# marl/l3embedding

Measured on AMD Instinct MI355X. Metric: AVC training pairs/sec (1s audio + 224x224 frame), higher is better.
Workload: dtype f32; 1 GPU; full cnn_L3_melspec2 AVC training step (audio+vision+fusion, fwd+bwd+Adam), batch 64 per GPU, global batch 64, fp32, inputs resident in HBM; global_batch=64, parallelism=dp1, fp32_conv=f4x4

## Files before the change

### include/l3hip.h

```cpp
#ifndef L3HIP_H
#define L3HIP_H

#include <stdint.h>

#ifdef __cplusplus
extern "C" {
#endif

#define L3_OK 0
#define L3_EINVAL (-1)
#define L3_EHIP (-2)
#define L3_ENOMEM (-3)
#define L3_ESTATE (-4)
#define L3_ECOMM (-5)

#define L3_MODEL_CNN_L3_ORIG 0
#define L3_MODEL_TINY_L3 1
#define L3_MODEL_CNN_L3_KAPREDBINPUTBN 2
#define L3_MODEL_CNN_L3_MELSPEC1 3
#define L3_MODEL_CNN_L3_MELSPEC2 4

typedef struct l3_engine l3_engine;

#define L3_DTYPE_F32 0
// ... 82 lines not shown
} l3_sample;
int l3_upload_batch_sampled(l3_engine *e, l3_clipbank *bank, const l3_sample *records, int n, int augment);
int l3_stage_batch_sampled(l3_engine *e, l3_clipbank *bank, const l3_sample *records, int n, int augment);
int l3_op_sample_batch(l3_clipbank *bank, const l3_sample *records, int n, int augment, uint8_t *out_u8, int16_t *out_i16,
                       double *gains);
int l3_step_forward(l3_engine *e, int training);
int l3_tower_step(l3_engine *e, int tower, int backward);
int l3_step_bucket_count(const l3_engine *e);
int l3_step_backward_bucket(l3_engine *e, int bucket);
int l3_step_update(l3_engine *e, float lr, float grad_scale);
int l3_step_resident(l3_engine *e, float lr);
int l3_step_results(l3_engine *e, float *loss, float *acc, float *probs, float *logits);
int l3_step_results_enqueue(l3_engine *e, int slot, int reduce);
int l3_step_results_wait(l3_engine *e, int slot, float *loss, float *acc);

int l3_replicas_upload(l3_engine *e, const float *video, const float *audio, const float *labels, int replicas);
int l3_replicas_upload_raw(l3_engine *e, const uint8_t *video_u8, const int16_t *audio_i16, const int32_t *labels_i32, int replicas);
int l3_replicas_upload_raw_aug(l3_engine *e, const uint8_t *video_u8, const int16_t *audio_i16, const int32_t *labels_i32,
                               const l3_augment_params *params, const double *u, int replicas);
int l3_replicas_stage_raw(l3_engine *e, const uint8_t *video_u8, const int16_t *audio_i16, const int32_t *labels_i32, int replicas);
int l3_replicas_stage_raw_aug(l3_engine *e, const uint8_t *video_u8, const int16_t *audio_i16, const int32_t *labels_i32,
                              const l3_augment_params *params, const double *u, int replicas);
int l3_step_replicas(l3_engine *e, float lr);
int l3_eval_replicas(l3_engine *e, float *loss, float *acc);

#define L3_COMM_ID_BYTES 128
int l3_comm_unique_id(void *id128);
int l3_comm_init(l3_engine *e, const void *id128, int world, int rank);
int l3_comm_destroy(l3_engine *e);
int l3_comm_info(const l3_engine *e, int *world, int *rank, char *library_path, int path_cap);
int l3_comm_version(void);
int l3_comm_allreduce_host(l3_engine *e, double *vals, int n, int op);
int l3_step_dp(l3_engine *e, float lr);
int l3_comm_timing(l3_engine *e, int on);
int l3_comm_timing_read(l3_engine *e, double *exposed_ms, double *span_ms, double *bucket_ms, int cap, int *steps);

int l3_grad_arena_dev(l3_engine *e, void **dev_ptr, int64_t *numel);
int l3_bucket_range(const l3_engine *e, int bucket, int64_t *offset, int64_t *numel);
int l3_bn_stats_pack_dev(l3_engine *e, void **send_dev, int64_t *numel);
int l3_bn_stats_replicas_dev(l3_engine *e, int world, void **gathered_dev);

int l3_embed_audio(l3_engine *e, const float *audio, int64_t n, int pool_h, int pool_w, float *out);
int l3_embed_vision(l3_engine *e, const float *video, int64_t n, int pool_h, int pool_w, float *out);
int64_t l3_embed_dim(const l3_engine *e, int vision, int pool_h, int pool_w);
int l3_embed_audio_frames(l3_engine *e, const float *samples, int64_t n_samples, const int64_t *table,
                          int64_t n_frames, int pool_h, int pool_w, float *out);
int l3_embed_audio_clips_resampled(l3_engine *e, const float *native, int64_t n_native, const int64_t *clips,
                                   int64_t n_clips, const double *half_window, int64_t n_window, int num_table,
                                   int64_t n_samples, const int64_t *table, int64_t n_frames, int pool_h, int pool_w,
                                   float *out);
int l3_embed_vision_frames(l3_engine *e, const uint8_t *pixels, int64_t n_bytes, const int64_t *table, int64_t n_frames,
                           int pool_h, int pool_w, float *out);

int l3_get_activation(l3_engine *e, const char *name, float *dst, int64_t numel);
int l3_activation_numel(l3_engine *e, const char *name, int64_t *numel);
int l3_sync(l3_engine *e);
int l3_profile_enable(l3_engine *e, int on);
int l3_set_tower_overlap(l3_engine *e, int on);
int l3_profile_read(l3_engine *e, int family, double *ms, int64_t *launches, double *flops);
int l3_profile_read_executed(l3_engine *e, int family, double *flops);
int l3_profile_read_bytes(l3_engine *e, int family, double *bytes);

#define L3_OP_BF16_STORED 2
#define L3_OP_BF16_STORED_OUT 3
int l3_op_conv2d_fwd_dt(int device, int dtype, const float *x, const float *w, const float *b, float *y,
                        int n, int h, int wd, int cin, int cout, int kh, int kw, int same);
int l3_op_conv2d_bwd_dt(int device, int dtype, const float *x, const float *w, const float *dy, float *dx,
                        float *dw, float *db, int n, int h, int wd, int cin, int cout, int kh, int kw, int same);
int l3_op_conv2d_fwd(int device, const float *x, const float *w, const float *b, float *y,
                     int n, int h, int wd, int cin, int cout, int kh, int kw, int same);
int l3_op_conv2d_bwd(int device, const float *x, const float *w, const float *dy,
                     float *dx, float *dw, float *db,
                     int n, int h, int wd, int cin, int cout, int kh, int kw, int same);
int l3_op_bn_relu_fwd(int device, const float *x, const float *gamma, const float *beta,
                      float *y, float *mean, float *var, int64_t rows, int c, int relu, int x_bf16);
int l3_op_bn_relu_bwd(int device, const float *x, const float *y, const float *dy,
                      const float *gamma, const float *beta, const float *mean, const float *var,
                      float *dx, float *dgamma, float *dbeta, int64_t rows, int c, int relu, int x_bf16);
int l3_op_bn_relu_pool2_fwd(int device, const float *x, const float *gamma, const float *beta, float *p,
                            float *mean, float *var, int n, int h, int wd, int c, int same, int relu_mode, int x_bf16);
int l3_op_bn_relu_pool2_bwd(int device, const float *x, const float *gamma, const float *beta, const float *dp,
                            float *dx, float *dgamma, float *dbeta, float *dbias, int n, int h, int wd, int c,
                            int same, int relu_mode, int x_bf16);
int l3_op_maxpool_fwd(int device, const float *x, float *y, int n, int h, int wd, int c,
                      int ph, int pw, int sh, int sw, int same);
int l3_op_maxpool_bwd(int device, const float *x, const float *dy, float *dx, int n, int h,
                      int wd, int c, int ph, int pw, int sh, int sw, int same);
int l3_op_frontend(int device, int model_type, const float *audio, int n, int db_max_scope, float *out);
int l3_op_frontend_form(int device, int model_type, int frontend, const float *audio, int n, float *out);
#define L3_FRONTEND_CFG_FIELDS 9
int l3_frontend_cfg(int t, int n_dft, int n_hop, int same, int n_mels, int32_t *cfg);
int l3_frontend_tables(const float *freq2mel, int n_mels, float *win, float *b1, float *b2, float *tw, int32_t *mel_start,
                       int32_t *mel_len, int32_t *mel_off, float *melw, int64_t melw_cap, int64_t *n_melw);
int l3_op_frontend_frames(int device, const float *audio, int b, int t, int n_dft, int n_hop, int pad_left, int n_frames,
                          float *frames, float *fe, float *fo, float *a1);
int l3_op_dft_twiddle(int device, const float *y, int frames, float *a2, float *nyq);
#define L3_SPEC_UNFOLDED 0
#define L3_SPEC_FOLDED 1
#define L3_SPEC_FACTORED 2
int l3_op_spec_to_features(int device, int layout, const float *spec, const float *nyq, int b, int n_frames, int n_dft, int n_mels,
                           const float *freq2mel, int flags, float *out);
int l3_op_dft_fused(int device, const float *audio, int b, int t, int n_hop, int pad_left, int n_frames, int n_mels,
                    const float *freq2mel, int flags, float *out);
int l3_op_db_normalize(int device, float *x, int b, int64_t per_sample, int batch_scope);
int l3_op_gather_frames(int device, const float *samples, int64_t n_samples, const int64_t *table,
                        int64_t n_frames, float *frames);
int l3_op_image_frames(int device, const uint8_t *pixels, int64_t n_bytes, const int64_t *table, int64_t n_frames,
                       uint8_t *out_u8, float *out_f32);
int l3_op_resample(int device, const float *x, int64_t n_in, int64_t sr_orig, int64_t sr_new, const double *half_window,
                   int64_t n_window, int num_table, int64_t t0, int64_t n_out, float *y);
int l3_op_resample_clips(int device, const float *x, int64_t n_in, const int64_t *clips, int64_t n_clips, int64_t sr_new,
                         const double *half_window, int64_t n_window, int num_table, int64_t n_samples, int copy_equal,
                         float *y);
int l3_op_bn_stats_from_partials(int device, const float *part, int nblk, int c, const float *pivot, int64_t rows,
                                 float eps, float *mean, float *var);
int l3_op_conv2d_fwd_stats(int device, int dtype, const float *x, const float *w, const float *b, float *y, float *part, int *nblk,
                           float *mean, float *var, int n, int h, int wd, int cin, int cout, int kh, int kw, int same,
                           int stat_mode);
int l3_op_conv2d_dgrad_bn_bwd(int device, int dtype, const float *dy, const float *w, const float *bn_x, const float *gamma,
                              const float *beta, const float *mean, const float *var, float *dx, float *part, int *nblk,
                              float *dgamma, float *dbeta, int n, int h, int wd, int cin, int cout, int kh, int kw, int same,
                              int relu, int64_t bn_rows);
int l3_op_first_block_bwd(int device, int form, int relu, const float *x, const float *gamma_in, const float *beta_in, const float *w,
                          const float *y, const float *gamma2, const float *beta2, const float *dA, float *mean_in, float *var_in,
                          float *xaug, float *mean2, float *var2, float *scale2, float *shift2, float *dgamma2, float *dbeta2,
                          float *coeffs, float *dY, float *gaug, float *dw, float *dbias, float *dgamma_in, float *dbeta_in, int n,
                          int h, int wd, int c, int cout);
int l3_op_first_conv_grads(int device, const float *gaug, const float *w, const float *gamma, const float *beta, float *dw,
                           float *dgamma, float *dbeta, float *dbias, int taps, int c, int co);
int l3_op_bn_relu_pool2_fwd_xwin(int device, const float *x, const float *gamma, const float *beta, float *p, float *mean,
                                 float *var, float *xwin, int n, int h, int wd, int c, int same, int relu_mode, int x_bf16);
int l3_op_preprocess(int device, const uint8_t *video_u8, int64_t nv, float *video,
                     const int16_t *audio_i16, int64_t na, float *audio);
int l3_op_augment_video(int device, const uint8_t *u8, int n, int h, int w, const l3_augment_params *params,
                        uint8_t *out_u8, float *out_f32);
int l3_op_augment_audio(int device, const int16_t *i16, int n, int t, const double *u, int16_t *out_i16, float *out_f32,
                        double *gains);

typedef struct l3_mlp l3_mlp;
int l3_mlp_create(int device, int D, int C, int batch, float weight_decay, uint64_t seed, l3_mlp **m);
void l3_mlp_destroy(l3_mlp *m);
int64_t l3_mlp_param_count(const l3_mlp *m);
int l3_mlp_set_data(l3_mlp *m, const float *X_train, const int32_t *y_train, int64_t n_train,
                    const float *X_valid, const int32_t *y_valid, int64_t n_valid);
int l3_mlp_epoch(l3_mlp *m, const int32_t *perm, float lr, int64_t t0, double *stats_out);
int l3_mlp_predict(l3_mlp *m, const float *X, int64_t n, float *probs_out);
int l3_mlp_get_weights(l3_mlp *m, float *dst, int64_t n);
int l3_mlp_set_weights(l3_mlp *m, const float *src, int64_t n);

int l3_op_mlp_dense_fwd(int device, const float *x, int64_t n_x, const int32_t *idx, int rows, int K, int N, const float *w,
                        const float *b, int relu, float *y);
int l3_op_mlp_dense_bwd_x(int device, const float *dy, const float *w, const float *h, int rows, int K, int N, float *dx);
int l3_op_mlp_wgrad(int device, const float *x, int64_t n_x, const int32_t *idx, int rows, int K, int N, const float *dy, float *dw,
                    float *db);
int l3_op_mlp_wgrad_adam(int device, const float *x, int64_t n_x, const int32_t *idx, int rows, int K, int N, const float *dy,
                         float *w, float *b, float *mw, float *vw, float *mb, float *vb, float weight_decay, float lr_t,
                         float *w2_out);
int l3_op_mlp_softmax_ce(int device, const float *z, const int32_t *labels, int rows, int C, float gscale, float *probs, float *dz,
                         float *ce, float *correct);
int l3_op_adam(int device, float *p, const float *g, float *m, float *v, int64_t n, int64_t n_l2, float l2x2, float lr_t);
int l3_op_adam_scaled(int device, float *p, const float *g, float *m, float *v, int64_t n, int64_t n_l2, float l2x2, float lr_t,
                      float b1, float b2, float eps, float gscale);
int l3_op_arena_fold(int device, float *acc, float *g, int64_t total, int64_t off, int64_t n, int mode);

int l3_op_head_dense_fwd(int device, const float *x, const float *w, const float *b, float *y, int B, int K, int N, int relu);
int l3_op_head_dense_bwd(int device, const float *x, const float *w, const float *dy, float *dw, float *db, float *dx, int B,
// ... 203 lines not shown
```

### l3embedding_amd/_lib.py

```python
import ctypes as C
import os

import numpy as np

from . import _build

MODEL_IDS = {
    'cnn_L3_orig': 0,
    'tiny_L3': 1,
    'cnn_L3_kapredbinputbn': 2,
    'cnn_L3_melspec1': 3,
    'cnn_L3_melspec2': 4,
}

FAMILIES = ('conv_fwd', 'conv_dgrad', 'conv_wgrad', 'elementwise', 'frontend', 'head', 'adam')


DTYPES = {'f32': 0, 'fp32': 0, 'float32': 0, 'bf16': 1}
FP32_CONV = {'f4x4': 0, 'f2x2': 1, 'f2x2_bf16x6': 2}
DP_MOVING = {'replicas': 0, 'rank_local': 1}
FRONTENDS = {'kapre': 0, 'minispec': 1}
OP_DTYPES = dict(DTYPES, bf16_stored=2, bf16_stored_out=3)


# ... 44 lines not shown
    'l3_reset_optimizer': (C.c_int, [C.c_void_p]),
    'l3_copy_state': (C.c_int, [C.c_void_p, C.c_void_p]),
    'l3_optimizer_steps': (C.c_int, [C.c_void_p, C.POINTER(C.c_int64), C.POINTER(C.c_int64)]),
    'l3_forward': (C.c_int, [C.c_void_p, C.c_void_p, C.c_void_p, C.c_int, C.c_void_p, C.c_void_p]),
    'l3_train_step': (C.c_int, [C.c_void_p, C.c_void_p, C.c_void_p, C.c_void_p, C.c_float,
                                C.POINTER(C.c_float), C.POINTER(C.c_float)]),
    'l3_eval_step': (C.c_int, [C.c_void_p, C.c_void_p, C.c_void_p, C.c_void_p,
                               C.POINTER(C.c_float), C.POINTER(C.c_float)]),
    'l3_upload_batch': (C.c_int, [C.c_void_p, C.c_void_p, C.c_void_p, C.c_void_p]),
    'l3_upload_batch_raw': (C.c_int, [C.c_void_p, C.c_void_p, C.c_void_p, C.c_void_p]),
    'l3_tower_step': (C.c_int, [C.c_void_p, C.c_int, C.c_int]),
    'l3_stage_batch_raw': (C.c_int, [C.c_void_p, C.c_void_p, C.c_void_p, C.c_void_p]),
    'l3_upload_batch_raw_aug': (C.c_int, [C.c_void_p, C.c_void_p, C.c_void_p, C.c_void_p, C.c_void_p, C.c_void_p]),
    'l3_stage_batch_raw_aug': (C.c_int, [C.c_void_p, C.c_void_p, C.c_void_p, C.c_void_p, C.c_void_p, C.c_void_p]),
    'l3_batch_gains': (C.c_int, [C.c_void_p, C.c_void_p]),
    'l3_clipbank_create': (C.c_int, [C.c_int, C.c_int64, C.c_int64, C.c_int, C.POINTER(C.c_void_p)]),
    'l3_clipbank_add': (C.c_int, [C.c_void_p, C.c_void_p, C.c_int, C.c_int, C.c_int, C.c_void_p, C.c_int64, C.c_int,
                                  C.POINTER(C.c_int)]),
    'l3_clipbank_info': (C.c_int, [C.c_void_p, C.c_int, C.c_void_p]),
    'l3_clipbank_audio': (C.c_int, [C.c_void_p, C.c_int, C.c_void_p]),
    'l3_clipbank_destroy': (None, [C.c_void_p]),
    'l3_upload_batch_sampled': (C.c_int, [C.c_void_p, C.c_void_p, C.c_void_p, C.c_int, C.c_int]),
    'l3_stage_batch_sampled': (C.c_int, [C.c_void_p, C.c_void_p, C.c_void_p, C.c_int, C.c_int]),
    'l3_op_sample_batch': (C.c_int, [C.c_void_p, C.c_void_p, C.c_int, C.c_int, C.c_void_p, C.c_void_p, C.c_void_p]),
    'l3_step_forward': (C.c_int, [C.c_void_p, C.c_int]),
    'l3_step_bucket_count': (C.c_int, [C.c_void_p]),
    'l3_step_backward_bucket': (C.c_int, [C.c_void_p, C.c_int]),
    'l3_step_update': (C.c_int, [C.c_void_p, C.c_float, C.c_float]),
    'l3_step_resident': (C.c_int, [C.c_void_p, C.c_float]),
    'l3_replicas_upload': (C.c_int, [C.c_void_p, C.c_void_p, C.c_void_p, C.c_void_p, C.c_int]),
    'l3_replicas_upload_raw': (C.c_int, [C.c_void_p, C.c_void_p, C.c_void_p, C.c_void_p, C.c_int]),
    'l3_replicas_stage_raw': (C.c_int, [C.c_void_p, C.c_void_p, C.c_void_p, C.c_void_p, C.c_int]),
    'l3_replicas_upload_raw_aug': (C.c_int, [C.c_void_p] * 6 + [C.c_int]),
    'l3_replicas_stage_raw_aug': (C.c_int, [C.c_void_p] * 6 + [C.c_int]),
    'l3_step_replicas': (C.c_int, [C.c_void_p, C.c_float]),
    'l3_eval_replicas': (C.c_int, [C.c_void_p, C.POINTER(C.c_float), C.POINTER(C.c_float)]),
    'l3_step_results': (C.c_int, [C.c_void_p, C.POINTER(C.c_float), C.POINTER(C.c_float), C.c_void_p, C.c_void_p]),
    'l3_step_results_enqueue': (C.c_int, [C.c_void_p, C.c_int, C.c_int]),
    'l3_step_results_wait': (C.c_int, [C.c_void_p, C.c_int, C.POINTER(C.c_float), C.POINTER(C.c_float)]),
    'l3_comm_unique_id': (C.c_int, [C.c_void_p]),
    'l3_comm_init': (C.c_int, [C.c_void_p, C.c_void_p, C.c_int, C.c_int]),
    'l3_comm_destroy': (C.c_int, [C.c_void_p]),
    'l3_comm_info': (C.c_int, [C.c_void_p, C.POINTER(C.c_int), C.POINTER(C.c_int), C.c_char_p, C.c_int]),
    'l3_comm_allreduce_host': (C.c_int, [C.c_void_p, C.POINTER(C.c_double), C.c_int, C.c_int]),
    'l3_step_dp': (C.c_int, [C.c_void_p, C.c_float]),
    'l3_comm_timing': (C.c_int, [C.c_void_p, C.c_int]),
    'l3_comm_timing_read': (C.c_int, [C.c_void_p, C.POINTER(C.c_double), C.POINTER(C.c_double), C.POINTER(C.c_double), C.c_int, C.POINTER(C.c_int)]),
    'l3_grad_arena_dev': (C.c_int, [C.c_void_p, C.POINTER(C.c_void_p), C.POINTER(C.c_int64)]),
    'l3_bucket_range': (C.c_int, [C.c_void_p, C.c_int, C.POINTER(C.c_int64), C.POINTER(C.c_int64)]),
    'l3_embed_audio': (C.c_int, [C.c_void_p, C.c_void_p, C.c_int64, C.c_int, C.c_int, C.c_void_p]),
    'l3_embed_vision': (C.c_int, [C.c_void_p, C.c_void_p, C.c_int64, C.c_int, C.c_int, C.c_void_p]),
    'l3_embed_dim': (C.c_int64, [C.c_void_p, C.c_int, C.c_int, C.c_int]),
    'l3_embed_audio_frames': (C.c_int, [C.c_void_p, C.c_void_p, C.c_int64, C.c_void_p, C.c_int64, C.c_int, C.c_int,
                                        C.c_void_p]),
    'l3_embed_audio_clips_resampled': (C.c_int, [C.c_void_p, C.c_void_p, C.c_int64, C.c_void_p, C.c_int64, C.c_void_p,
                                                 C.c_int64, C.c_int, C.c_int64, C.c_void_p, C.c_int64, C.c_int, C.c_int,
                                                 C.c_void_p]),
    'l3_embed_audio_frames_dev': (C.c_int, [C.c_void_p, C.c_void_p, C.c_int64, C.c_void_p, C.c_int64, C.c_int, C.c_int,
                                            C.c_void_p, C.c_int64]),
    'l3_embed_audio_clips_resampled_dev': (C.c_int, [C.c_void_p, C.c_void_p, C.c_int64, C.c_void_p, C.c_int64, C.c_void_p,
                                                     C.c_int64, C.c_int, C.c_int64, C.c_void_p, C.c_int64, C.c_int, C.c_int,
                                                     C.c_void_p, C.c_int64]),
    'l3_embed_vision_frames': (C.c_int, [C.c_void_p, C.c_void_p, C.c_int64, C.c_void_p, C.c_int64, C.c_int, C.c_int,
                                         C.c_void_p]),
    'l3_embed_vision_frames_dev': (C.c_int, [C.c_void_p, C.c_void_p, C.c_int64, C.c_void_p, C.c_int64, C.c_int, C.c_int,
                                             C.c_void_p, C.c_int64]),
    'l3_get_activation': (C.c_int, [C.c_void_p, C.c_char_p, C.c_void_p, C.c_int64]),
    'l3_activation_numel': (C.c_int, [C.c_void_p, C.c_char_p, C.POINTER(C.c_int64)]),
    'l3_sync': (C.c_int, [C.c_void_p]),
    'l3_profile_enable': (C.c_int, [C.c_void_p, C.c_int]),
    'l3_set_tower_overlap': (C.c_int, [C.c_void_p, C.c_int]),
    'l3_profile_read_executed': (C.c_int, [C.c_void_p, C.c_int, C.POINTER(C.c_double)]),
    'l3_profile_read_bytes': (C.c_int, [C.c_void_p, C.c_int, C.POINTER(C.c_double)]),
    'l3_profile_read': (C.c_int, [C.c_void_p, C.c_int, C.POINTER(C.c_double), C.POINTER(C.c_int64),
                                  C.POINTER(C.c_double)]),
    'l3_op_conv2d_fwd': (C.c_int, [C.c_int, C.c_void_p, C.c_void_p, C.c_void_p, C.c_void_p] + [C.c_int] * 8),
    'l3_op_conv2d_fwd_dt': (C.c_int, [C.c_int, C.c_int, C.c_void_p, C.c_void_p, C.c_void_p, C.c_void_p] + [C.c_int] * 8),
    'l3_op_conv2d_bwd_dt': (C.c_int, [C.c_int, C.c_int] + [C.c_void_p] * 6 + [C.c_int] * 8),
    'l3_op_conv2d_bwd': (C.c_int, [C.c_int] + [C.c_void_p] * 6 + [C.c_int] * 8),
    'l3_op_bn_relu_fwd': (C.c_int, [C.c_int] + [C.c_void_p] * 6 + [C.c_int64, C.c_int, C.c_int, C.c_int]),
    'l3_op_bn_relu_bwd': (C.c_int, [C.c_int] + [C.c_void_p] * 10 + [C.c_int64, C.c_int, C.c_int, C.c_int]),
    'l3_op_bn_relu_pool2_fwd': (C.c_int, [C.c_int] + [C.c_void_p] * 6 + [C.c_int] * 7),
    'l3_op_bn_relu_pool2_bwd': (C.c_int, [C.c_int] + [C.c_void_p] * 8 + [C.c_int] * 7),
    'l3_op_maxpool_fwd': (C.c_int, [C.c_int, C.c_void_p, C.c_void_p] + [C.c_int] * 9),
    'l3_op_maxpool_bwd': (C.c_int, [C.c_int, C.c_void_p, C.c_void_p, C.c_void_p] + [C.c_int] * 9),
    'l3_op_frontend': (C.c_int, [C.c_int, C.c_int, C.c_void_p, C.c_int, C.c_int, C.c_void_p]),
    'l3_op_frontend_form': (C.c_int, [C.c_int, C.c_int, C.c_int, C.c_void_p, C.c_int, C.c_void_p]),
    'l3_spectrogram_shape': (C.c_int, [C.c_void_p, C.c_void_p, C.c_void_p]),
    'l3_audio_spectrograms': (C.c_int, [C.c_void_p, C.c_void_p, C.c_int64, C.c_void_p, C.c_int64, C.c_void_p]),
    'l3_embed_audio_spec': (C.c_int, [C.c_void_p, C.c_void_p, C.c_int64, C.c_int, C.c_int, C.c_void_p]),
    'l3_embed_audio_spec_dev': (C.c_int, [C.c_void_p, C.c_void_p, C.c_int64, C.c_int, C.c_int, C.c_void_p, C.c_int64]),
    'l3_tower_dim': (C.c_int, [C.c_void_p, C.c_int]),
    'l3_tower_features': (C.c_int, [C.c_void_p, C.c_int, C.c_void_p, C.c_int64, C.c_void_p]),
    'l3_tower_features_dev': (C.c_int, [C.c_void_p, C.c_int, C.c_void_p, C.c_int64, C.c_void_p, C.c_int64]),
    'l3_tower_features_sampled_dev': (C.c_int, [C.c_void_p, C.c_void_p, C.c_void_p, C.c_int64, C.c_void_p, C.c_void_p, C.c_int64]),
    'l3_pairs_create': (C.c_int, [C.c_int, C.c_int, C.c_int, C.c_int, C.POINTER(C.c_void_p)]),
    'l3_pairs_destroy': (None, [C.c_void_p]),
    'l3_pairs_set_head': (C.c_int, [C.c_void_p] * 5),
    'l3_pairs_set_vision': (C.c_int, [C.c_void_p, C.c_void_p, C.c_int64]),
    'l3_pairs_set_audio': (C.c_int, [C.c_void_p, C.c_void_p, C.c_int64]),
    'l3_pairs_set_vision_dev': (C.c_int, [C.c_void_p, C.c_void_p, C.c_int64, C.c_int64]),
    'l3_pairs_set_audio_dev': (C.c_int, [C.c_void_p, C.c_void_p, C.c_int64, C.c_int64]),
    'l3_pairs_matrix': (C.c_int, [C.c_void_p] + [C.c_int64] * 4 + [C.c_int, C.c_void_p]),
    'l3_pairs_list': (C.c_int, [C.c_void_p, C.c_void_p, C.c_void_p, C.c_int64, C.c_void_p]),
    'l3_pairs_ranks': (C.c_int, [C.c_void_p] * 7),
    'l3_pairs_time': (C.c_int, [C.c_void_p, C.c_int, C.c_int64, C.c_int, C.POINTER(C.c_double)]),
    'l3_op_project': (C.c_int, [C.c_int, C.c_void_p, C.c_void_p, C.c_void_p, C.c_int64, C.c_int, C.c_int, C.c_void_p]),
    'l3_op_pair_margins': (C.c_int, [C.c_int, C.c_void_p, C.c_void_p, C.c_void_p, C.c_float, C.c_int64, C.c_int64, C.c_int, C.c_void_p]),
    'l3_frontend_cfg': (C.c_int, [C.c_int] * 5 + [C.c_void_p]),
    'l3_frontend_tables': (C.c_int, [C.c_void_p, C.c_int] + [C.c_void_p] * 8 + [C.c_int64, C.POINTER(C.c_int64)]),
    'l3_op_frontend_frames': (C.c_int, [C.c_int, C.c_void_p] + [C.c_int] * 6 + [C.c_void_p] * 4),
    'l3_op_dft_twiddle': (C.c_int, [C.c_int, C.c_void_p, C.c_int, C.c_void_p, C.c_void_p]),
    'l3_op_spec_to_features': (C.c_int, [C.c_int, C.c_int, C.c_void_p, C.c_void_p] + [C.c_int] * 4 + [C.c_void_p, C.c_int, C.c_void_p]),
    'l3_op_dft_fused': (C.c_int, [C.c_int, C.c_void_p] + [C.c_int] * 6 + [C.c_void_p, C.c_int, C.c_void_p]),
    'l3_op_db_normalize': (C.c_int, [C.c_int, C.c_void_p, C.c_int, C.c_int64, C.c_int]),
    'l3_op_gather_frames': (C.c_int, [C.c_int, C.c_void_p, C.c_int64, C.c_void_p, C.c_int64, C.c_void_p]),
    'l3_op_image_frames': (C.c_int, [C.c_int, C.c_void_p, C.c_int64, C.c_void_p, C.c_int64, C.c_void_p, C.c_void_p]),
    'l3_op_resample': (C.c_int, [C.c_int, C.c_void_p, C.c_int64, C.c_int64, C.c_int64, C.c_void_p, C.c_int64, C.c_int,
                                 C.c_int64, C.c_int64, C.c_void_p]),
    'l3_op_resample_clips': (C.c_int, [C.c_int, C.c_void_p, C.c_int64, C.c_void_p, C.c_int64, C.c_int64, C.c_void_p, C.c_int64,
                                       C.c_int, C.c_int64, C.c_int, C.c_void_p]),
    'l3_op_bn_stats_from_partials': (C.c_int, [C.c_int, C.c_void_p, C.c_int, C.c_int, C.c_void_p, C.c_int64, C.c_float,
                                               C.c_void_p, C.c_void_p]),
    'l3_op_conv2d_fwd_stats': (C.c_int, [C.c_int, C.c_int] + [C.c_void_p] * 5 + [C.POINTER(C.c_int), C.c_void_p, C.c_void_p] +
                               [C.c_int] * 9),
    'l3_op_conv2d_dgrad_bn_bwd': (C.c_int, [C.c_int, C.c_int] + [C.c_void_p] * 9 + [C.POINTER(C.c_int), C.c_void_p, C.c_void_p] +
                                  [C.c_int] * 9 + [C.c_int64]),
    'l3_op_first_block_bwd': (C.c_int, [C.c_int] * 3 + [C.c_void_p] * 24 + [C.c_int] * 5),
    'l3_op_first_conv_grads': (C.c_int, [C.c_int] + [C.c_void_p] * 8 + [C.c_int] * 3),
    'l3_op_bn_relu_pool2_fwd_xwin': (C.c_int, [C.c_int] + [C.c_void_p] * 7 + [C.c_int] * 7),
    'l3_op_preprocess': (C.c_int, [C.c_int, C.c_void_p, C.c_int64, C.c_void_p, C.c_void_p, C.c_int64, C.c_void_p]),
    'l3_op_augment_video': (C.c_int, [C.c_int, C.c_void_p, C.c_int, C.c_int, C.c_int, C.c_void_p, C.c_void_p, C.c_void_p]),
    'l3_op_augment_audio': (C.c_int, [C.c_int, C.c_void_p, C.c_int, C.c_int, C.c_void_p, C.c_void_p, C.c_void_p, C.c_void_p]),
    'l3_mlp_create': (C.c_int, [C.c_int, C.c_int, C.c_int, C.c_int, C.c_float, C.c_uint64, C.POINTER(C.c_void_p)]),
    'l3_mlp_destroy': (None, [C.c_void_p]),
    'l3_mlp_param_count': (C.c_int64, [C.c_void_p]),
    'l3_mlp_set_data': (C.c_int, [C.c_void_p, C.c_void_p, C.c_void_p, C.c_int64, C.c_void_p, C.c_void_p, C.c_int64]),
    'l3_mlp_epoch': (C.c_int, [C.c_void_p, C.c_void_p, C.c_float, C.c_int64, C.POINTER(C.c_double)]),
    'l3_mlp_predict': (C.c_int, [C.c_void_p, C.c_void_p, C.c_int64, C.c_void_p]),
    'l3_mlp_get_weights': (C.c_int, [C.c_void_p, C.c_void_p, C.c_int64]),
    'l3_mlp_set_weights': (C.c_int, [C.c_void_p, C.c_void_p, C.c_int64]),
    'l3_op_mlp_dense_fwd': (C.c_int, [C.c_int, C.c_void_p, C.c_int64, C.c_void_p, C.c_int, C.c_int, C.c_int, C.c_void_p,
                                      C.c_void_p, C.c_int, C.c_void_p]),
    'l3_op_mlp_dense_bwd_x': (C.c_int, [C.c_int, C.c_void_p, C.c_void_p, C.c_void_p, C.c_int, C.c_int, C.c_int, C.c_void_p]),
    'l3_op_mlp_wgrad': (C.c_int, [C.c_int, C.c_void_p, C.c_int64, C.c_void_p, C.c_int, C.c_int, C.c_int, C.c_void_p,
                                  C.c_void_p, C.c_void_p]),
    'l3_op_mlp_wgrad_adam': (C.c_int, [C.c_int, C.c_void_p, C.c_int64, C.c_void_p, C.c_int, C.c_int, C.c_int, C.c_void_p]
                             + [C.c_void_p] * 6 + [C.c_float, C.c_float, C.c_void_p]),
    'l3_op_mlp_softmax_ce': (C.c_int, [C.c_int, C.c_void_p, C.c_void_p, C.c_int, C.c_int, C.c_float] + [C.c_void_p] * 4),
    'l3_op_adam': (C.c_int, [C.c_int] + [C.c_void_p] * 4 + [C.c_int64, C.c_int64, C.c_float, C.c_float]),
    'l3_op_adam_scaled': (C.c_int, [C.c_int] + [C.c_void_p] * 4 + [C.c_int64, C.c_int64] + [C.c_float] * 6),
    'l3_op_arena_fold': (C.c_int, [C.c_int, C.c_void_p, C.c_void_p, C.c_int64, C.c_int64, C.c_int64, C.c_int]),
    'l3_op_head_dense_fwd': (C.c_int, [C.c_int] + [C.c_void_p] * 4 + [C.c_int] * 4),
    'l3_op_head_dense_bwd': (C.c_int, [C.c_int] + [C.c_void_p] * 6 + [C.c_int] * 3),
    'l3_op_softmax_ce2': (C.c_int, [C.c_int, C.c_void_p, C.c_void_p, C.c_int, C.c_float] + [C.c_void_p] * 3),
    'l3_op_sumsq': (C.c_int, [C.c_int, C.c_void_p, C.c_int64, C.c_void_p, C.c_void_p, C.c_int, C.c_int, C.c_void_p]),
    'l3_op_bn_moving_update': (C.c_int, [C.c_int, C.c_int, C.c_void_p, C.c_void_p, C.c_int64] + [C.c_void_p] * 4
                               + [C.c_int64, C.c_int, C.c_int64, C.c_float, C.c_int, C.c_int64, C.c_void_p, C.c_int64]),
    'l3_svm_create': (C.c_int, [C.c_int, C.POINTER(C.c_void_p)]),
    'l3_svm_destroy': (None, [C.c_void_p]),
    'l3_svm_set_data': (C.c_int, [C.c_void_p, C.c_void_p, C.c_int64, C.c_int]),
    'l3_svm_fit': (C.c_int, [C.c_void_p, C.c_void_p, C.c_double, C.c_double, C.c_int64, C.c_int] + [C.c_void_p] * 3
                   + [C.c_int] + [C.c_void_p] * 5),
    'l3_svm_fit_costs': (C.c_int, [C.c_void_p, C.c_void_p, C.c_void_p, C.c_double, C.c_int64, C.c_int] + [C.c_void_p] * 3
                         + [C.c_int] + [C.c_void_p] * 5),
    'l3_svm_cv_decision': (C.c_int, [C.c_void_p, C.c_void_p, C.c_int] + [C.c_void_p] * 8),
# ... 689 lines not shown
    for k in ('mean2', 'var2', 'scale2', 'shift2', 'dgamma2', 'dbeta2'):
        out[k] = np.empty(co, f32)
    coeffs = np.empty((3, co), f32) if form != 'explicit' else None
    dY = np.empty_like(y) if form == 'explicit' else None
    out.update(gaug=np.empty((9, c + 1, co), f32), dw=np.empty((3, 3, c, co), f32), dbias=np.empty(co, f32),
               dgamma_in=np.empty(c, f32), dbeta_in=np.empty(c, f32))
    names = ('mean_in', 'var_in', 'xaug', 'mean2', 'var2', 'scale2', 'shift2', 'dgamma2', 'dbeta2')
    tail = ('gaug', 'dw', 'dbias', 'dgamma_in', 'dbeta_in')
    check(lib.l3_op_first_block_bwd(device, FIRST_BLOCK_FORMS[form], int(relu), _ptr(x), _ptr(vin[0]), _ptr(vin[1]), _ptr(w), _ptr(y),
                                    _ptr(v2[0]), _ptr(v2[1]), _ptr(dA), *([_ptr(out[k]) for k in names] + [_ptr(coeffs), _ptr(dY)] +
                                                                          [_ptr(out[k]) for k in tail] + [n, h, wd, c, co])))
    if dY is not None:
        out['dY'] = dY
    else:
        out['cA'], out['cB'], out['cC'] = coeffs
    return out


def op_first_conv_grads(gaug, w, gamma, beta, want_dbias=True, device=0):
    lib = load()
    gaug, w, gamma, beta = _f32(gaug), _f32(w), _f32(gamma), _f32(beta)
    taps, c, co = w.shape
    assert gaug.shape == (taps, c + 1, co) and gamma.shape == (c,) and beta.shape == (c,)
    dw = np.empty_like(w)
    dg, db = np.empty(c, np.float32), np.empty(c, np.float32)
    dbias = np.empty(co, np.float32) if want_dbias else None
    check(lib.l3_op_first_conv_grads(device, _ptr(gaug), _ptr(w), _ptr(gamma), _ptr(beta), _ptr(dw), _ptr(dg), _ptr(db), _ptr(dbias),
                                     taps, c, co))
    return dw, dg, db, dbias


def op_bn_relu_fwd(x, gamma, beta, relu, device=0, x_bf16=False, out_bf16=False):
    lib = load()
    x = _f32(x)
    c = x.shape[-1]
    rows = x.size // c
    y = np.empty_like(x)
    mean, var = np.empty((c,), np.float32), np.empty((c,), np.float32)
    check(lib.l3_op_bn_relu_fwd(device, _ptr(x), _ptr(_f32(gamma)), _ptr(_f32(beta)), _ptr(y), _ptr(mean),
                                _ptr(var), rows, c, int(relu), int(x_bf16) | (4 if out_bf16 else 0)))
    return y, mean, var


def op_bn_relu_bwd(x, y, dy, gamma, mean, var, relu, device=0, beta=None, x_bf16=False, out_bf16=False):
    lib = load()
    x, y, dy = _f32(x), _f32(y), _f32(dy)
    c = x.shape[-1]
    rows = x.size // c
    dx = np.empty_like(x)
    dg, db = np.empty((c,), np.float32), np.empty((c,), np.float32)
    check(lib.l3_op_bn_relu_bwd(device, _ptr(x), _ptr(y), _ptr(dy), _ptr(_f32(gamma)), _ptr(_f32(beta)), _ptr(_f32(mean)),
                                _ptr(_f32(var)), _ptr(dx), _ptr(dg), _ptr(db), rows, c, int(relu), int(x_bf16) | (4 if out_bf16 else 0)))
    return dx, dg, db


def op_bn_relu_pool2_fwd(x, gamma, beta, same, device=0, relu_mode=1, x_bf16=False, want_xwin=False, out_bf16=False):
    lib = load()
    flags = int(x_bf16) | (4 if out_bf16 else 0)
    x = _f32(x)
    n, h, wd, c = x.shape
    p = np.empty((n, _pool_out(h, 2, 2, same), _pool_out(wd, 2, 2, same), c), np.float32)
    mean, var = np.empty((c,), np.float32), np.empty((c,), np.float32)
    if want_xwin:
        xwin = np.empty_like(p)
        check(lib.l3_op_bn_relu_pool2_fwd_xwin(device, _ptr(x), _ptr(_f32(gamma)), _ptr(_f32(beta)), _ptr(p), _ptr(mean), _ptr(var),
                                               _ptr(xwin), n, h, wd, c, int(same), int(relu_mode), flags))
        return p, mean, var, xwin
    check(lib.l3_op_bn_relu_pool2_fwd(device, _ptr(x), _ptr(_f32(gamma)), _ptr(_f32(beta)), _ptr(p), _ptr(mean),
                                      _ptr(var), n, h, wd, c, int(same), int(relu_mode), flags))
    return p, mean, var


def op_bn_relu_pool2_bwd(x, gamma, beta, dp, same, device=0, relu_mode=1, x_bf16=False, out_bf16=False):
    lib = load()
    x, dp = _f32(x), _f32(dp)
    n, h, wd, c = x.shape
    dx = np.empty_like(x)
    dg, db, dbias = (np.empty((c,), np.float32) for _ in range(3))
    check(lib.l3_op_bn_relu_pool2_bwd(device, _ptr(x), _ptr(_f32(gamma)), _ptr(_f32(beta)), _ptr(dp), _ptr(dx),
                                      _ptr(dg), _ptr(db), _ptr(dbias), n, h, wd, c, int(same), int(relu_mode), int(x_bf16) | (4 if out_bf16 else 0)))
    return dx, dg, db, dbias


def _pool_out(h, p, s, same):
    return -(-h // s) if same else (h - p) // s + 1


def op_maxpool_fwd(x, ph, pw, sh, sw, same, device=0):
    lib = load()
    x = _f32(x)
    n, h, wd, c = x.shape
    y = np.empty((n, _pool_out(h, ph, sh, same), _pool_out(wd, pw, sw, same), c), np.float32)
    check(lib.l3_op_maxpool_fwd(device, _ptr(x), _ptr(y), n, h, wd, c, ph, pw, sh, sw, int(same)))
    return y


def op_maxpool_bwd(x, dy, ph, pw, sh, sw, same, device=0):
    lib = load()
    x, dy = _f32(x), _f32(dy)
    n, h, wd, c = x.shape
    dx = np.empty_like(x)
    check(lib.l3_op_maxpool_bwd(device, _ptr(x), _ptr(dy), _ptr(dx), n, h, wd, c, ph, pw, sh, sw, int(same)))
    return dx


def op_bn_stats_from_partials(part, pivot, rows, eps=1e-3, device=0):
    lib = load()
    part, pivot = _f32(part), _f32(pivot)
    nblk, two, c = part.shape
    assert two == 2 and pivot.shape == (c,)
    mean, var = np.empty(c, np.float32), np.empty(c, np.float32)
    check(lib.l3_op_bn_stats_from_partials(device, _ptr(part), nblk, c, _ptr(pivot), int(rows), float(eps), _ptr(mean), _ptr(var)))
    return mean, var


def op_frontend(model_type, audio, db_max_scope='sample', device=0):
    lib = load()
    a = _f32(audio)
    n = a.shape[0]
    probe = {'cnn_L3_orig': (257, 197), 'tiny_L3': (257, 198), 'cnn_L3_kapredbinputbn': (257, 197),
             'cnn_L3_melspec1': (128, 199), 'cnn_L3_melspec2': (256, 199)}[model_type]
    out = np.empty((n, probe[0], probe[1], 1), np.float32)
    check(lib.l3_op_frontend(device, MODEL_IDS[model_type], _ptr(a), n, 0 if db_max_scope == 'sample' else 1, _ptr(out)))
    return out


def op_frontend_form(model_type, audio, frontend='minispec', device=0):
    lib = load()
    a = _f32(audio)
    n = a.shape[0]
    f, frames = {'cnn_L3_orig': (257, 197), 'tiny_L3': (257, 198), 'cnn_L3_kapredbinputbn': (257, 197),
                 'cnn_L3_melspec1': (128, 199), 'cnn_L3_melspec2': (256, 199)}[model_type]
    if frontend == 'minispec':
        frames = 199
    out = np.empty((n, f, frames, 1), np.float32)
    check(lib.l3_op_frontend_form(device, MODEL_IDS[model_type], FRONTENDS[frontend], _ptr(a), n, _ptr(out)))
    return out


FRONTEND_CFG_FIELDS = ('n_frames', 'pad_left', 'n_freq', 'ncols_pad', 'ke', 'ko', 'nc', 'N1', 'N2')
SPEC_LAYOUTS = dict(unfolded=0, folded=1, factored=2)


def frontend_cfg(t, n_dft, n_hop, same, n_mels=0):
    v = np.zeros(len(FRONTEND_CFG_FIELDS), np.int32)
    check(load().l3_frontend_cfg(int(t), int(n_dft), int(n_hop), int(bool(same)), int(n_mels), _ptr(v)))
    return dict(zip(FRONTEND_CFG_FIELDS, (int(x) for x in v)))


def frontend_tables(n_mels=0, freq2mel=None):
    f32 = np.float32
    out = dict(win=np.empty(2048, f32), b1=np.empty((32, 64), f32), b2=np.empty((128, 64), f32), tw=np.empty((64, 32, 2), f32))
    fb = _f32(freq2mel)
    assert fb is None or fb.shape == (1025, n_mels)
    st, ln, of = (np.zeros(n_mels, np.int32) for _ in range(3))
    cap = 1025 * max(n_mels, 1)
    melw = np.empty(cap, f32)
    n = C.c_int64(0)
    check(load().l3_frontend_tables(_ptr(fb), int(n_mels), _ptr(out['win']), _ptr(out['b1']), _ptr(out['b2']), _ptr(out['tw']), _ptr(st),
                                    _ptr(ln), _ptr(of), _ptr(melw), cap, C.byref(n)))
    if n_mels:
        out.update(mel_start=st, mel_len=ln, mel_off=of, melw=melw[:n.value].copy())
    return out


def op_frontend_frames(audio, n_dft, n_hop, pad_left, n_frames, device=0):
# ... 1368 lines not shown
```

### l3embedding_amd/csrc/bn_fused.hip

```cpp
#include "kernels.h"
#include "device_common.h"

namespace l3 {



__device__ __forceinline__ void store_quad(void* base, int64_t q, f32x4 v, int obf) {
    if (obf) {
        bf16x4 h;
        h[0] = (__bf16)v.x; h[1] = (__bf16)v.y; h[2] = (__bf16)v.z; h[3] = (__bf16)v.w;
        __builtin_nontemporal_store(h, reinterpret_cast<bf16x4*>(base) + q);
    } else {
        __builtin_nontemporal_store(v, reinterpret_cast<f32x4*>(base) + q);
    }
}

template <bool XBF>
__device__ __forceinline__ f32x4 load_quad(const void* base, int64_t q) {
    if constexpr (XBF) {
        const u32x2 r = __builtin_nontemporal_load(reinterpret_cast<const u32x2*>(base) + q);
        return f32x4{__uint_as_float(r.x << 16), __uint_as_float(r.x & 0xffff0000u), __uint_as_float(r.y << 16),
                     __uint_as_float(r.y & 0xffff0000u)};
    } else {
        return __builtin_nontemporal_load(reinterpret_cast<const f32x4*>(base) + q);
// ... 236 lines not shown
template <bool XBF, bool WIN>
__global__ __launch_bounds__(FB) void bn_relu_pool2_fwd_kernel(const void* __restrict__ x, const f32x4* scale, const f32x4* shift,
                                                              void* __restrict__ p, Pool2Geom g, int mode, int obf, void* __restrict__ xwin) {
    constexpr int U = 2;
    const int64_t total = (int64_t)g.N * g.Ho * g.Wo * g.C4;
    const int c4 = (int)threadIdx.x % g.C4;
    const f32x4 sc = scale[c4], sh = shift[c4];
    const int64_t stride = (int64_t)gridDim.x * (FB * U);
    for (int64_t q = (int64_t)blockIdx.x * (FB * U) + threadIdx.x; q < total; q += stride) {
        f32x4 xs[U][4];
        int64_t po[U], wo_[U];
        bool w1[U], h1[U], live[U];
#pragma unroll
        for (int u = 0; u < U; ++u) {
            live[u] = q + u * FB < total;
            int n = 0, ho = 0, wo = 0;
            pool_index(g, live[u] ? q + u * FB : q, g.Ho, g.Wo, n, ho, wo);
            const int h0 = 2 * ho, w0 = 2 * wo;
            h1[u] = h0 + 1 < g.H; w1[u] = w0 + 1 < g.W;
            const int64_t base = ((int64_t)(n * g.H + h0) * g.W + w0) * g.C4 + c4;
            const int64_t dw = w1[u] ? g.C4 : 0, dh = h1[u] ? (int64_t)g.W * g.C4 : 0;
            xs[u][0] = load_quad<XBF>(x, base); xs[u][1] = load_quad<XBF>(x, base + dw);
            xs[u][2] = load_quad<XBF>(x, base + dh); xs[u][3] = load_quad<XBF>(x, base + dh + dw);
            po[u] = (int64_t)n * g.out_bs4 + ((int64_t)ho * g.Wo + wo) * g.C4 + c4;
            wo_[u] = ((int64_t)(n * g.Ho + ho) * g.Wo + wo) * g.C4 + c4;
        }
#pragma unroll
        for (int u = 0; u < U; ++u) {
            if (!live[u]) continue;
            f32x4 x00 = xs[u][0], x01 = xs[u][1], x10 = xs[u][2], x11 = xs[u][3];
            const bool h1ok = h1[u], w1ok = w1[u];
            if (mode == 2) { x00 = relu4(x00); x01 = relu4(x01); x10 = relu4(x10); x11 = relu4(x11); }
            const f32x4 v00 = bn_pre(x00, sc, sh), v01 = bn_pre(x01, sc, sh);
            const f32x4 v10 = bn_pre(x10, sc, sh), v11 = bn_pre(x11, sc, sh);
            f32x4 m;
            m.x = fmaxf(fmaxf(v00.x, v01.x), fmaxf(v10.x, v11.x));
            m.y = fmaxf(fmaxf(v00.y, v01.y), fmaxf(v10.y, v11.y));
            m.z = fmaxf(fmaxf(v00.z, v01.z), fmaxf(v10.z, v11.z));
            m.w = fmaxf(fmaxf(v00.w, v01.w), fmaxf(v10.w, v11.w));
            if (mode == 1) m = relu4(m);
            store_quad(p, po[u], m, obf);
            if constexpr (WIN) {
                const f32x4 r00 = mode == 1 ? relu4(v00) : v00, r01 = mode == 1 ? relu4(v01) : v01;
                const f32x4 r10 = mode == 1 ? relu4(v10) : v10, r11 = mode == 1 ? relu4(v11) : v11;
                const bool ok11 = h1ok && w1ok;
                f32x4 xw;
#define L3_WIN(comp)                                                                                  \
    {                                                                                                 \
        const int k = argmax4(r00.comp, r01.comp, r10.comp, r11.comp, w1ok, h1ok, ok11);              \
        xw.comp = k == 0 ? x00.comp : k == 1 ? x01.comp : k == 2 ? x10.comp : x11.comp;               \
    }
                L3_WIN(x) L3_WIN(y) L3_WIN(z) L3_WIN(w)
#undef L3_WIN
                store_quad(xwin, wo_[u], xw, XBF ? 1 : 0);
            }
        }
    }
}

static Pool2Geom make_pool2(int N, int H, int W, int C, int Ho, int Wo, int64_t out_batch_stride) {
    Pool2Geom g;
    g.N = N; g.H = H; g.W = W; g.C4 = C / 4; g.Ho = Ho; g.Wo = Wo;
    g.Hc = (H + 1) / 2; g.Wc = (W + 1) / 2;
    g.out_bs4 = out_batch_stride / 4;
    g.lgC4 = 0;
    while ((1 << g.lgC4) < g.C4) ++g.lgC4;
    g.small = (int64_t)N * g.Hc * g.Wc < ((int64_t)1 << 31) && (int64_t)N * H * W < ((int64_t)1 << 31);
    return g;
}

void bn_relu_pool2_fwd(const float* x, const float* scale, const float* shift, float* p, int N, int H, int W, int C,
                       int Ho, int Wo, int64_t out_batch_stride, int mode, hipStream_t s, int out_bf16, int x_bf16, void* xwin) {
    const Pool2Geom g = make_pool2(N, H, W, C, Ho, Wo, out_batch_stride);
    const int64_t total = (int64_t)N * Ho * Wo * g.C4;
    int64_t nb = (total + FB * 2 - 1) / (FB * 2);
    if (nb > 65536) nb = 65536;
    if (nb < 1) nb = 1;
    auto k = xwin != nullptr ? (x_bf16 ? bn_relu_pool2_fwd_kernel<true, true> : bn_relu_pool2_fwd_kernel<false, true>)
                             : (x_bf16 ? bn_relu_pool2_fwd_kernel<true, false> : bn_relu_pool2_fwd_kernel<false, false>);
    hipLaunchKernelGGL(k, dim3((int)nb), dim3(FB), 0, s, (const void*)x, reinterpret_cast<const f32x4*>(scale),
                       reinterpret_cast<const f32x4*>(shift), (void*)p, g, mode, out_bf16, xwin);
}

struct BwdCoef {
    float *A, *B, *Cc;
};

template <bool POOL, bool XBF, bool DYBF>
__global__ __launch_bounds__(FB) void bn_bwd_reduce_fast_kernel(const void* x, const void* dy, const f32x4* scale,
                                                               const f32x4* shift, const f32x4* mean,
                                                               const f32x4* var, float* part, int64_t n4,
                                                               Pool2Geom g, float eps, int relu) {
    const int64_t q0 = (int64_t)blockIdx.x * FB + threadIdx.x;
    const int c4 = (int)(q0 % g.C4);
    const f32x4 sc = scale[c4], sh = shift[c4], mu = mean[c4];
    const f32x4 vv = var[c4];
    const f32x4 rs = {rsqrtf(vv.x + eps), rsqrtf(vv.y + eps), rsqrtf(vv.z + eps), rsqrtf(vv.w + eps)};
    f32x4 a0 = {0.f, 0.f, 0.f, 0.f}, a1 = {0.f, 0.f, 0.f, 0.f};
    const int64_t stride = (int64_t)gridDim.x * FB;
    if constexpr (!POOL) {
        for (int64_t q = q0; q < n4; q += stride) {
            f32x4 xv = load_quad<XBF>(x, q);
            f32x4 d = load_quad<DYBF>(dy, q);
            if (relu == 1) {
                const f32x4 pre = bn_pre(xv, sc, sh);
                d.x = pre.x > 0.f ? d.x : 0.f; d.y = pre.y > 0.f ? d.y : 0.f;
                d.z = pre.z > 0.f ? d.z : 0.f; d.w = pre.w > 0.f ? d.w : 0.f;
            } else if (relu == 2) {
                xv = relu4(xv);
            }
            a0 += d;
            a1 += d * ((xv - mu) * rs);
        }
    } else {
        const int64_t total = (int64_t)g.N * g.Ho * g.Wo * g.C4;
        for (int64_t q = q0; q < total; q += stride) {
            int n, ho, wo;
            pool_index(g, q, g.Ho, g.Wo, n, ho, wo);
            const int h0 = 2 * ho, w0 = 2 * wo;
            const bool h1ok = h0 + 1 < g.H, w1ok = w0 + 1 < g.W;
            const int64_t base = ((int64_t)(n * g.H + h0) * g.W + w0) * g.C4 + c4;
            const int64_t dw = w1ok ? g.C4 : 0, dh = h1ok ? (int64_t)g.W * g.C4 : 0;
            f32x4 x00 = load_quad<XBF>(x, base), x01 = load_quad<XBF>(x, base + dw), x10 = load_quad<XBF>(x, base + dh),
                  x11 = load_quad<XBF>(x, base + dh + dw);
            if (relu == 2) { x00 = relu4(x00); x01 = relu4(x01); x10 = relu4(x10); x11 = relu4(x11); }
            f32x4 p00 = bn_pre(x00, sc, sh), p01 = bn_pre(x01, sc, sh), p10 = bn_pre(x10, sc, sh),
                  p11 = bn_pre(x11, sc, sh);
            const float gate = relu == 2 ? -INFINITY : 0.f;
            if (relu != 2) { p00 = relu4(p00); p01 = relu4(p01); p10 = relu4(p10); p11 = relu4(p11); }
            const f32x4 dp = load_quad<DYBF>(dy, (int64_t)n * g.out_bs4 + ((int64_t)ho * g.Wo + wo) * g.C4 + c4);
            const bool ok11 = h1ok && w1ok;
#define L3_RED(comp)                                                                                      \
    {                                                                                                     \
        const int k = argmax4(p00.comp, p01.comp, p10.comp, p11.comp, w1ok, h1ok, ok11);                  \
        const float pk = k == 0 ? p00.comp : k == 1 ? p01.comp : k == 2 ? p10.comp : p11.comp;            \
        const float xk = k == 0 ? x00.comp : k == 1 ? x01.comp : k == 2 ? x10.comp : x11.comp;            \
        const float d = pk > gate ? dp.comp : 0.f;                                                        \
        a0.comp += d;                                                                                     \
        a1.comp += d * ((xk - mu.comp) * rs.comp);                                                        \
    }
            L3_RED(x) L3_RED(y) L3_RED(z) L3_RED(w)
#undef L3_RED
        }
    }
    block_write_partials(a0, a1, part, g.C4);
}

struct BwdFinal {
    const float* gamma;
    const float* mean;
    const float* var;
    float *dgamma, *dbeta, *A, *B, *Cc;
    double inv_n;
    float eps;
    int training;
    __device__ void operator()(int c, double s0, double s1) const {
        dbeta[c] = (float)s0;
        dgamma[c] = (float)s1;
        const double rstd = 1.0 / sqrt((double)var[c] + (double)eps);
        const double gr = (double)gamma[c] * rstd;
        A[c] = (float)gr;
        if (training) {
            B[c] = (float)(-gr * rstd * s1 * inv_n);
            Cc[c] = (float)(gr * (-s0 * inv_n + (double)mean[c] * rstd * s1 * inv_n));
        } else {
            B[c] = 0.f;
            Cc[c] = 0.f;
        }
    }
};

template <bool POOL, bool XBF, bool DYBF>
__global__ __launch_bounds__(FB) void bn_bwd_apply_fast_kernel(const void* x, const void* dy, const f32x4* scale,
                                                              const f32x4* shift, const f32x4* cA, const f32x4* cB,
                                                              const f32x4* cC, void* dx, float* part, int64_t n4,
                                                              Pool2Geom g, int relu, int obf) {
    const int64_t q0 = (int64_t)blockIdx.x * FB + threadIdx.x;
    const int c4 = (int)(q0 % g.C4);
    const f32x4 sc = scale[c4], sh = shift[c4], A = cA[c4], B = cB[c4], Cc = cC[c4];
    f32x4 a0 = {0.f, 0.f, 0.f, 0.f};
    const int64_t stride = (int64_t)gridDim.x * FB;
    if constexpr (!POOL) {
        for (int64_t q = q0; q < n4; q += stride) {
            const f32x4 xr = load_quad<XBF>(x, q);
            f32x4 xv = xr;
            f32x4 d = load_quad<DYBF>(dy, q);
            if (relu == 1) {
                const f32x4 pre = bn_pre(xv, sc, sh);
                d.x = pre.x > 0.f ? d.x : 0.f; d.y = pre.y > 0.f ? d.y : 0.f;
                d.z = pre.z > 0.f ? d.z : 0.f; d.w = pre.w > 0.f ? d.w : 0.f;
            } else if (relu == 2) {
                xv = relu4(xv);
            }
            f32x4 o = A * d + (B * xv + Cc);
            if (relu == 2) {
                o.x = xr.x > 0.f ? o.x : 0.f; o.y = xr.y > 0.f ? o.y : 0.f;
                o.z = xr.z > 0.f ? o.z : 0.f; o.w = xr.w > 0.f ? o.w : 0.f;
            }
            store_quad(dx, q, o, obf);
            a0 += o;
        }
    } else {
        constexpr int U = XBF ? 2 : 1;
        const int64_t total = (int64_t)g.N * g.Hc * g.Wc * g.C4;
        for (int64_t q = (int64_t)blockIdx.x * (FB * U) + threadIdx.x; q < total; q += stride * U) {
            f32x4 rs[U][4], dps[U];
            int64_t bases[U];
            bool w1[U], h1[U], lives[U], on[U];
#pragma unroll
            for (int u = 0; u < U; ++u) {
                on[u] = q + u * FB < total;
                int n, hc, wc;
                pool_index(g, on[u] ? q + u * FB : q, g.Hc, g.Wc, n, hc, wc);
                const int h0 = 2 * hc, w0 = 2 * wc;
                h1[u] = h0 + 1 < g.H; w1[u] = w0 + 1 < g.W;
                lives[u] = hc < g.Ho && wc < g.Wo;
                const int64_t base = ((int64_t)(n * g.H + h0) * g.W + w0) * g.C4 + c4;
                const int64_t dw = w1[u] ? g.C4 : 0, dh = h1[u] ? (int64_t)g.W * g.C4 : 0;
                bases[u] = base;
                rs[u][0] = load_quad<XBF>(x, base); rs[u][1] = load_quad<XBF>(x, base + dw);
                rs[u][2] = load_quad<XBF>(x, base + dh); rs[u][3] = load_quad<XBF>(x, base + dh + dw);
                dps[u] = f32x4{0.f, 0.f, 0.f, 0.f};
                if (lives[u]) dps[u] = load_quad<DYBF>(dy, (int64_t)n * g.out_bs4 + ((int64_t)hc * g.Wo + wc) * g.C4 + c4);
            }
#pragma unroll
            for (int u = 0; u < U; ++u) {
                if (!on[u]) continue;
                const bool h1ok = h1[u], w1ok = w1[u], live = lives[u];
                const int64_t base = bases[u];
                const int64_t dw = w1ok ? g.C4 : 0, dh = h1ok ? (int64_t)g.W * g.C4 : 0;
                const f32x4 r00 = rs[u][0], r01 = rs[u][1], r10 = rs[u][2], r11 = rs[u][3];
                f32x4 x00 = r00, x01 = r01, x10 = r10, x11 = r11;
                if (relu == 2) { x00 = relu4(x00); x01 = relu4(x01); x10 = relu4(x10); x11 = relu4(x11); }
                f32x4 d00 = {0.f, 0.f, 0.f, 0.f}, d01 = d00, d10 = d00, d11 = d00;
                if (live) {
                    f32x4 p00 = bn_pre(x00, sc, sh), p01 = bn_pre(x01, sc, sh), p10 = bn_pre(x10, sc, sh),
                          p11 = bn_pre(x11, sc, sh);
                    const float gate = relu == 2 ? -INFINITY : 0.f;
                    if (relu != 2) { p00 = relu4(p00); p01 = relu4(p01); p10 = relu4(p10); p11 = relu4(p11); }
                    const f32x4 dp = dps[u];
                    const bool ok11 = h1ok && w1ok;
#define L3_APP(comp)                                                                                      \
    {                                                                                                     \
        const int k = argmax4(p00.comp, p01.comp, p10.comp, p11.comp, w1ok, h1ok, ok11);                  \
        const float pk = k == 0 ? p00.comp : k == 1 ? p01.comp : k == 2 ? p10.comp : p11.comp;            \
        const float d = pk > gate ? dp.comp : 0.f;                                                        \
        d00.comp = k == 0 ? d : 0.f;                                                                      \
        d01.comp = k == 1 ? d : 0.f;                                                                      \
        d10.comp = k == 2 ? d : 0.f;                                                                      \
        d11.comp = k == 3 ? d : 0.f;                                                                      \
    }
                    L3_APP(x) L3_APP(y) L3_APP(z) L3_APP(w)
#undef L3_APP
                }
                auto gate2 = [&](f32x4 o, f32x4 r) {
                    if (relu == 2) {
                        o.x = r.x > 0.f ? o.x : 0.f; o.y = r.y > 0.f ? o.y : 0.f;
                        o.z = r.z > 0.f ? o.z : 0.f; o.w = r.w > 0.f ? o.w : 0.f;
                    }
                    return o;
                };
                const f32x4 o00 = gate2(A * d00 + (B * x00 + Cc), r00);
                store_quad(dx, base, o00, obf);
                a0 += o00;
                if (w1ok) {
                    const f32x4 o = gate2(A * d01 + (B * x01 + Cc), r01);
                    store_quad(dx, base + dw, o, obf);
                    a0 += o;
                }
                if (h1ok) {
                    const f32x4 o = gate2(A * d10 + (B * x10 + Cc), r10);
                    store_quad(dx, base + dh, o, obf);
                    a0 += o;
                }
                if (h1ok && w1ok) {
                    const f32x4 o = gate2(A * d11 + (B * x11 + Cc), r11);
                    store_quad(dx, base + dh + dw, o, obf);
                    a0 += o;
                }
            }
        }
    }
    if (part != nullptr) block_write_partials(a0, a0, part, g.C4);
}

struct SumFinal {
    float* out;
    __device__ void operator()(int c, double s0, double) const { out[c] = (float)s0; }
};

void bn_bwd_fast(const float* x, const float* scale, const float* shift, const float* mean, const float* var,
                 const float* gamma, const float* dy, int pooled, int N, int H, int W, int C, int Ho, int Wo,
                 int64_t dy_batch_stride, float* dx, float* dgamma, float* dbeta, float* dbias, float* scratch,
                 float eps, int relu, int training, hipStream_t s, int dx_bf16, int x_bf16, int dy_bf16,
                 const float* ready_part, int ready_blocks) {
    const int64_t rows = (int64_t)N * H * W;
    const int64_t n4 = rows * (C / 4);
    Pool2Geom g = make_pool2(N, H, W, C, pooled ? Ho : H, pooled ? Wo : W, pooled ? dy_batch_stride : (int64_t)H * W * C);
    float* part = scratch;
    float* cA = scratch + (size_t)FAST_MAX_BLOCKS * 2 * C;
    float* cB = cA + C;
    float* cC = cB + C;
    const void* xv = (const void*)x;
    const void* dyv = (const void*)dy;
    const f32x4* sc4 = reinterpret_cast<const f32x4*>(scale);
    const f32x4* sh4 = reinterpret_cast<const f32x4*>(shift);
    const int64_t work_r = pooled ? (int64_t)N * Ho * Wo * (C / 4) : n4;
    const int nb_r = fast_blocks(work_r);
    const int variant = (pooled ? 4 : 0) | (x_bf16 ? 2 : 0) | (dy_bf16 ? 1 : 0);
    using ReduceFn = void (*)(const void*, const void*, const f32x4*, const f32x4*, const f32x4*, const f32x4*, float*, int64_t,
                              Pool2Geom, float, int);
    static const ReduceFn reduce_fns[8] = {
        bn_bwd_reduce_fast_kernel<false, false, false>, bn_bwd_reduce_fast_kernel<false, false, true>,
        bn_bwd_reduce_fast_kernel<false, true, false>,  bn_bwd_reduce_fast_kernel<false, true, true>,
        bn_bwd_reduce_fast_kernel<true, false, false>,  bn_bwd_reduce_fast_kernel<true, false, true>,
        bn_bwd_reduce_fast_kernel<true, true, false>,   bn_bwd_reduce_fast_kernel<true, true, true>};
    if (ready_part != nullptr) {
        launch_fast_final(BwdFinal{gamma, mean, var, dgamma, dbeta, cA, cB, cC, 1.0 / (double)rows, eps, training}, ready_part,
                          ready_blocks, C, s);
    } else {
        hipLaunchKernelGGL(reduce_fns[variant], dim3(nb_r), dim3(FB), 0, s, xv, dyv, sc4, sh4, reinterpret_cast<const f32x4*>(mean),
                           reinterpret_cast<const f32x4*>(var), part, n4, g, eps, relu);
        launch_fast_final(BwdFinal{gamma, mean, var, dgamma, dbeta, cA, cB, cC, 1.0 / (double)rows, eps, training}, part,
                          nb_r, C, s);
    }
    if (dx == nullptr) return;
    const int64_t work_a = pooled ? (int64_t)N * g.Hc * g.Wc * (C / 4) : n4;
    const int nb_a = fast_blocks(work_a);
    float* part2 = dbias ? part : nullptr;
    using ApplyFn = void (*)(const void*, const void*, const f32x4*, const f32x4*, const f32x4*, const f32x4*, const f32x4*, void*,
                             float*, int64_t, Pool2Geom, int, int);
    static const ApplyFn apply_fns[8] = {
        bn_bwd_apply_fast_kernel<false, false, false>, bn_bwd_apply_fast_kernel<false, false, true>,
        bn_bwd_apply_fast_kernel<false, true, false>,  bn_bwd_apply_fast_kernel<false, true, true>,
        bn_bwd_apply_fast_kernel<true, false, false>,  bn_bwd_apply_fast_kernel<true, false, true>,
        bn_bwd_apply_fast_kernel<true, true, false>,   bn_bwd_apply_fast_kernel<true, true, true>};
    hipLaunchKernelGGL(apply_fns[variant], dim3(nb_a), dim3(FB), 0, s, xv, dyv, sc4, sh4, reinterpret_cast<const f32x4*>(cA),
                       reinterpret_cast<const f32x4*>(cB), reinterpret_cast<const f32x4*>(cC), (void*)dx, part2, n4, g, relu,
                       dx_bf16);
    if (dbias) launch_fast_final(SumFinal{dbias}, part, nb_a, C, s);
}

}
```

### l3embedding_amd/csrc/elementwise.hip

```cpp
#include <algorithm>

#include "kernels.h"

namespace l3 {

static constexpr int RED_BLOCK = 256;
static constexpr int RED_MAX_BLOCKS = 1024;
static constexpr int SMALLC_MAX = 16;

static inline int red_blocks(int64_t rows, int C) {
    int rows_per_pass = (C % 4 == 0 && C >= 4 && C <= 1024) ? (RED_BLOCK / (C / 4) > 0 ? RED_BLOCK / (C / 4) : 1) : RED_BLOCK;
    int64_t b = (rows + (int64_t)rows_per_pass * 16 - 1) / ((int64_t)rows_per_pass * 16);
    if (b < 1) b = 1;
    if (b > RED_MAX_BLOCKS) b = RED_MAX_BLOCKS;
    return (int)b;
}

size_t colreduce_scratch_floats(int64_t rows, int C) {
    const size_t a = (size_t)red_blocks(rows, C) * 2 * (size_t)(C < 4 ? 4 : C) + 64;
    const size_t b = bn_fast_ok(C) ? bn_fast_scratch_floats(C) : 0;
    return a > b ? a : b;
}

template <class F>
// ... 446 lines not shown
}
typedef float gp4 __attribute__((ext_vector_type(4)));
__device__ __forceinline__ void gp_scan(const float* __restrict__ xb, int P, int C, int pg, float best[4], int arg[4]) {
#pragma unroll
    for (int e = 0; e < 4; ++e) {
        best[e] = -INFINITY;
        arg[e] = 0x7fffffff;
    }
    for (int p = pg; p < P; p += 16) {
        const gp4 v = *reinterpret_cast<const gp4*>(xb + (size_t)p * C);
#pragma unroll
        for (int e = 0; e < 4; ++e)
            if (v[e] > best[e] || arg[e] == 0x7fffffff) {
                best[e] = v[e];
                arg[e] = p;
            }
    }
}
__device__ __forceinline__ void gp_merge(float (*sb)[64], int (*sa)[64], int pg, int cq, float best[4], int arg[4]) {
#pragma unroll
    for (int e = 0; e < 4; ++e) {
        sb[pg][cq * 4 + e] = best[e];
        sa[pg][cq * 4 + e] = arg[e];
    }
    __syncthreads();
    if (pg == 0) {
#pragma unroll
        for (int e = 0; e < 4; ++e) {
            float b = best[e];
            int a = arg[e];
            for (int k = 1; k < 16; ++k) {
                const float vb = sb[k][cq * 4 + e];
                const int va = sa[k][cq * 4 + e];
                if (vb > b || (vb == b && va < a)) {
                    b = vb;
                    a = va;
                }
            }
            sb[0][cq * 4 + e] = b;
            sa[0][cq * 4 + e] = a;
        }
    }
    __syncthreads();
}
__global__ __launch_bounds__(256) void global_maxpool_fwd_kernel(const float* __restrict__ x, float* __restrict__ y, int P,
                                                                 int C, int64_t out_batch_stride) {
    __shared__ float sb[16][64];
    __shared__ int sa[16][64];
    const int cb = blockIdx.x % (C / 64), n = blockIdx.x / (C / 64);
    const int cq = threadIdx.x & 15, pg = threadIdx.x >> 4;
    float best[4];
    int arg[4];
    gp_scan(x + (size_t)n * P * C + cb * 64 + cq * 4, P, C, pg, best, arg);
    gp_merge(sb, sa, pg, cq, best, arg);
    if (threadIdx.x < 64) y[(size_t)n * out_batch_stride + cb * 64 + threadIdx.x] = sb[0][threadIdx.x];
}
__global__ __launch_bounds__(256) void global_maxpool_bwd_kernel(const float* __restrict__ x, const float* __restrict__ dy,
                                                                 float* __restrict__ dx, int P, int C,
                                                                 int64_t out_batch_stride) {
    __shared__ float sb[16][64];
    __shared__ int sa[16][64];
    const int cb = blockIdx.x % (C / 64), n = blockIdx.x / (C / 64);
    const int cq = threadIdx.x & 15, pg = threadIdx.x >> 4;
    float best[4];
    int arg[4];
    const size_t base = (size_t)n * P * C + cb * 64 + cq * 4;
    gp_scan(x + base, P, C, pg, best, arg);
    gp_merge(sb, sa, pg, cq, best, arg);
    const gp4 d = *reinterpret_cast<const gp4*>(dy + (size_t)n * out_batch_stride + cb * 64 + cq * 4);
    int am[4];
#pragma unroll
    for (int e = 0; e < 4; ++e) am[e] = sa[0][cq * 4 + e];
    for (int p = pg; p < P; p += 16) {
        gp4 o;
#pragma unroll
        for (int e = 0; e < 4; ++e) o[e] = p == am[e] ? d[e] : 0.f;
        *reinterpret_cast<gp4*>(dx + base + (size_t)p * C) = o;
    }
}
static bool is_global_pool(const PoolGeom& g) {
    return g.Ho == 1 && g.Wo == 1 && g.padT == 0 && g.padL == 0 && g.ph == g.H && g.pw == g.W && g.C % 64 == 0 &&
           g.out_batch_stride % 4 == 0;
}

void maxpool_fwd(const float* x, float* y, const PoolGeom& g, hipStream_t s) {
    if (is_global_pool(g)) {
        hipLaunchKernelGGL(global_maxpool_fwd_kernel, dim3(g.N * (g.C / 64)), dim3(256), 0, s, x, y, g.H * g.W, g.C,
                           (int64_t)g.out_batch_stride);
        return;
    }
    const int64_t total = (int64_t)g.N * g.Ho * g.Wo * g.C;
    hipLaunchKernelGGL(maxpool_fwd_kernel, dim3(ew_blocks(total)), dim3(256), 0, s, x, y, g);
}
__global__ __launch_bounds__(256) void maxpool_bwd_kernel(const float* x, const float* dy, float* dx, PoolGeom g) {
    const int64_t total = (int64_t)g.N * g.Ho * g.Wo * g.C;
    for (int64_t i = (int64_t)blockIdx.x * 256 + threadIdx.x; i < total; i += (int64_t)gridDim.x * 256) {
        const int c = (int)(i % g.C);
        int64_t r = i / g.C;
        const int wo = (int)(r % g.Wo);
        r /= g.Wo;
        const int ho = (int)(r % g.Ho);
        const int n = (int)(r / g.Ho);
        const int h0 = ho * g.sh - g.padT, w0 = wo * g.sw - g.padL;
        float best = -INFINITY;
        int ba = -1, bb = -1;
        for (int a = 0; a < g.ph; ++a) {
            const int h = h0 + a;
            if ((unsigned)h >= (unsigned)g.H) continue;
            for (int b = 0; b < g.pw; ++b) {
                const int w = w0 + b;
                if ((unsigned)w >= (unsigned)g.W) continue;
                const float v = x[((size_t)(n * g.H + h) * g.W + w) * g.C + c];
                if (ba < 0 || v > best) { best = v; ba = a; bb = b; }
            }
        }
        const float d = dy[(size_t)n * g.out_batch_stride + ((size_t)ho * g.Wo + wo) * g.C + c];
        for (int a = 0; a < g.ph; ++a) {
            const int h = h0 + a;
            if ((unsigned)h >= (unsigned)g.H) continue;
            for (int b = 0; b < g.pw; ++b) {
                const int w = w0 + b;
                if ((unsigned)w >= (unsigned)g.W) continue;
                dx[((size_t)(n * g.H + h) * g.W + w) * g.C + c] = (a == ba && b == bb) ? d : 0.f;
            }
        }
    }
}
void maxpool_bwd(const float* x, const float* dy, float* dx, const PoolGeom& g, hipStream_t s) {
    if (is_global_pool(g)) {
        hipLaunchKernelGGL(global_maxpool_bwd_kernel, dim3(g.N * (g.C / 64)), dim3(256), 0, s, x, dy, dx, g.H * g.W,
                           g.C, (int64_t)g.out_batch_stride);
        return;
    }
    const bool covers = (g.Ho - 1) * g.sh - g.padT + g.ph >= g.H && (g.Wo - 1) * g.sw - g.padL + g.pw >= g.W &&
                        g.sh == g.ph && g.sw == g.pw;
    if (!covers) (void)hipMemsetAsync(dx, 0, (size_t)g.N * g.H * g.W * g.C * sizeof(float), s);
    const int64_t total = (int64_t)g.N * g.Ho * g.Wo * g.C;
    hipLaunchKernelGGL(maxpool_bwd_kernel, dim3(ew_blocks(total)), dim3(256), 0, s, x, dy, dx, g);
}

__global__ __launch_bounds__(256) void bn_xhat_ones_kernel(const float* __restrict__ x, const float* __restrict__ mean,
                                                           const float* __restrict__ var, float eps, float* __restrict__ xa,
                                                           int64_t rows, int C) {
    const int C1 = C + 1;
    const int64_t total = rows * C1;
    for (int64_t i = (int64_t)blockIdx.x * 256 + threadIdx.x; i < total; i += (int64_t)gridDim.x * 256) {
        const int c = (int)(i % C1);
        const int64_t r = i / C1;
        xa[i] = c == C ? 1.f : (x[r * C + c] - mean[c]) * (1.f / sqrtf(var[c] + eps));
    }
}
void bn_xhat_ones(const float* x, const float* mean, const float* var, float eps, float* xa, int64_t rows, int C,
                  hipStream_t s) {
    hipLaunchKernelGGL(bn_xhat_ones_kernel, dim3(ew_blocks(rows * (C + 1))), dim3(256), 0, s, x, mean, var, eps, xa, rows, C);
}

__global__ __launch_bounds__(256) void first_conv_grads_kernel(const float* __restrict__ gaug, const float* __restrict__ w,
                                                               const float* __restrict__ gamma, const float* __restrict__ beta,
                                                               float* __restrict__ dw, float* __restrict__ dgamma,
                                                               float* __restrict__ dbeta, float* __restrict__ dbias, int taps,
                                                               int C, int Co) {
    __shared__ double red[2][256];
    const int t = threadIdx.x;
    const int C1 = C + 1;
    for (int i = t; i < taps * C * Co; i += 256) {
        const int co = i % Co, ci = (i / Co) % C, tap = i / (Co * C);
// ... 324 lines not shown
```

### l3embedding_amd/csrc/engine.hip

```cpp
#include <hip/hip_runtime.h>
#include "knobs.h"

#include <cmath>
#include <cstdio>
#include <cstdlib>
#include <cstring>
#include <map>
#include <string>
#include <vector>

#include "../../include/l3hip.h"
#include "comm.h"
#include "conv_path.h"
#include "featprep.h"
#include "kernels.h"

namespace {

using namespace l3;

static thread_local std::string g_create_error;

constexpr float BN_EPS = 1e-3f;
constexpr float BN_MOMENTUM = 0.99f;
constexpr float L2_WEIGHT = 1e-5f;
constexpr float ADAM_B1 = 0.9f, ADAM_B2 = 0.999f, ADAM_EPS = 1e-8f;
constexpr int AUDIO_T = 48000;

enum ParamKind { PK_KERNEL, PK_BIAS, PK_GAMMA, PK_BETA, PK_MMEAN, PK_MVAR, PK_CONST };
enum OpKind { OP_CONV, OP_BN, OP_RELU, OP_POOL, OP_FLATTEN };
enum Family { F_CONV_FWD, F_CONV_DGRAD, F_CONV_WGRAD, F_ELEMWISE, F_FRONTEND, F_HEAD, F_ADAM, F_COUNT };

struct Tensor {
    float* d = nullptr;
    float* g = nullptr;
    int N = 0, H = 0, W = 0, C = 0;
    int64_t batch_stride = 0;
    bool alias = false;
    bool d_bf16 = false, g_bf16 = false;
    int64_t numel() const { return (int64_t)N * H * W * C; }
    int64_t rows() const { return (int64_t)N * H * W; }
};

struct Param {
    std::string name;
    int ndim = 0;
    int64_t shape[4] = {1, 1, 1, 1};
    bool trainable = false;
    int kind = 0;
    int64_t numel = 0;
    int bucket = 0;
    float* d = nullptr;
    float* g = nullptr;
};

enum FirstWgrad { FW_NONE, FW_AUG, FW_AUG_DEFERRED };
struct ConvPlan {
    ConvStorage st;
    ConvFwdPath fwd;
    int stat_mode = 0;
    FirstWgrad aug = FW_NONE;
    ConvWgradPath wgrad;
    bool colsum = false;
    ConvDgradPath dgrad;
    int bwd_bn = -1;
    double fwd_bytes = 0.0, wg_bytes = 0.0, dg_bytes = 0.0;
};
enum BnStats { BS_PARTIALS, BS_FAST, BS_PLAIN, BS_MOVING };
enum BnBwd { BB_BY_FIRST_CONV, BB_FAST_POOLED, BB_FAST, BB_FAST_DEFERRED, BB_PLAIN };
struct BnPlan {
    BnStats stats = BS_MOVING;
    int stat_blocks = 0;
    BnBwd bwd = BB_PLAIN;
    int bwd_blocks = 0;
    double fwd_bytes = 0.0, bwd_bytes = 0.0;
};

struct Op {
    OpKind kind;
    std::string name;
    int in = 0, out = 0;
    int block = 0, bucket = 0;
    int kh = 0, kw = 0, cout = 0;
    bool same = false;
    ConvGeom geom{};
    ConvGeom dgeom{};
    int p_kernel = -1, p_bias = -1;
    float* wflip = nullptr;
    float *wino_uf = nullptr, *wino_ud = nullptr;
    int in_bn = -1;
    bool fused_first = false;
    bool defer_apply = false;
    int bn_defer = -1;
    float *xaug = nullptr, *gaug = nullptr;
    ConvGeom ageom{};
    int bn_follow = -1;
    bool need_dx = true;
    int dy_to_bn = -1;
    float* xwin = nullptr;
    int p_gamma = -1, p_beta = -1, p_mmean = -1, p_mvar = -1;
    bool fused_relu = false;
    bool prerelu = false;
    int fuse_pool = -1;
    int bias_param = -1;
    bool fused_into_bn = false;
    bool bias_by_bn = false;
    float *mean = nullptr, *var = nullptr, *scale = nullptr, *shift = nullptr;
    float *biased_mean = nullptr, *biased_var = nullptr;
    PoolGeom pg{};
    ConvPlan cp{};
    BnPlan bp{};
};

struct Tower {
    std::string prefix;
    std::vector<Tensor> t;
    std::vector<Op> ops;
    int nblocks = 0;
    int emb_conv_op = -1;
    bool training = false;
};

struct FrontendDef {
    int n_dft, n_hop, same, n_mels, sqrt_out, db, loglambda;
    const char* layer_name;
};

struct ProfRec {
    int family;
    hipEvent_t a, b;
    double flops;
    double executed;
    double bytes;
    const char* tag;
};

}

struct l3_engine {
    l3_config cfg{};
    int B = 0;
    hipStream_t stream = nullptr;
    bool own_stream = false;
    hipStream_t side = nullptr;
    hipEvent_t ev_fork = nullptr, ev_join = nullptr;
    float *red_scratch2 = nullptr, *wg_scratch2 = nullptr;
    float *stat_scratch = nullptr, *stat_scratch2 = nullptr;
    size_t stat_max = 0;
    float* w4_tail = nullptr;
    bool overlap = true;
    BnMovingEntry* bn_table = nullptr;
    int bn_table_n = 0, bn_table_max_c = 0;
    std::string err;
    l3::DeviceBufs bufs;

    std::vector<Param> params;
    std::map<std::string, int> pindex;
    float *arena_p = nullptr, *arena_g = nullptr, *arena_m = nullptr, *arena_v = nullptr;
    int64_t n_train = 0;
    struct Segment { int64_t off, n; bool l2; };
    std::vector<Segment> segments;
    struct Bucket { int64_t off, n; };
    std::vector<Bucket> buckets;
    int64_t adam_t = 0;
    int64_t bn_step = 0;

    Tower vis, aud;
    FrontendDef fe{};
    FrontendCfg fcfg{};
    int p_real = -1, p_imag = -1, p_mel = -1;
    bool consts_dirty = true;
    float *wdft = nullptr, *melw = nullptr, *frames = nullptr, *spec = nullptr, *smax = nullptr;
    bool dft_consts_done = false;
    float *dft_win = nullptr, *dft_b1 = nullptr, *dft_b2 = nullptr, *dft_tw = nullptr, *dft_y = nullptr, *dft_a2 = nullptr, *dft_nyq = nullptr;
    int *mel_start = nullptr, *mel_len = nullptr, *mel_off = nullptr;
    int64_t melw_cap = 0;

    float *video = nullptr, *audio = nullptr, *labels = nullptr;
    l3::BatchFeed feed;
    float* res_host = nullptr;
    float* res_sum = nullptr;
    bool res_reduced[2] = {false, false};
    bool res_pending[2] = {false, false};
    hipEvent_t ev_res[2] = {nullptr, nullptr};
    hipEvent_t ev_res_a = nullptr, ev_res_b = nullptr;
    hipEvent_t ev_step[2] = {nullptr, nullptr};
    bool ev_step_set[2] = {false, false};
    int64_t steps_enqueued = 0;
// ... 704 lines not shown
            for (size_t ci = 0; ci < tw->ops.size(); ++ci) {
                Op& cv = tw->ops[ci];
                if (cv.kind == OP_CONV && conv_first_ok(cv.geom) && cv.bn_follow >= 0 && cv.bias_by_bn &&
                    (int)ci != tw->emb_conv_op)
                    tw->t[cv.out].d_bf16 = true;
            }
    auto t_floats = [](const Tensor& t, bool bf16) { return bf16 ? (size_t)(t.numel() + 1) / 2 : (size_t)t.numel(); };
    size_t red_max = 1024, wg_max = 16;
    size_t& stat_max = e->stat_max;
    for (int ti = 0; ti < 2; ++ti) {
        Tower& tw = ti == 0 ? e->vis : e->aud;
        tw.t[0].d = ti == 0 ? e->video : nullptr;
        if (ti == 1) {
            if ((rc = dev_alloc_t(e, &tw.t[0].d, (size_t)tw.t[0].numel()))) return rc;
        }
        const int64_t concat_off = ti == 0 ? 0 : e->nv;
        for (size_t oi = 0; oi < tw.ops.size(); ++oi) {
            Op& op = tw.ops[oi];
            Tensor& y = tw.t[op.out];
            const bool last = oi + 1 == tw.ops.size();
            if (last) {
                y.d = e->h0 + concat_off;
                y.g = e->dh0 + concat_off;
                y.batch_stride = D;
                y.alias = true;
                if (op.kind == OP_POOL) op.pg.out_batch_stride = D;
            } else if ((op.kind == OP_BN && op.fuse_pool >= 0) || (op.kind == OP_RELU && op.fused_into_bn)) {
                if (op.kind == OP_BN) {
                    bool wanted = false;
                    for (size_t ci = 0; ci < tw.ops.size(); ++ci)
                        if (tw.ops[ci].kind == OP_CONV && tw.ops[ci].dy_to_bn == (int)oi) wanted = true;
                    const Tensor& pl = tw.t[tw.ops[op.fuse_pool].out];
                    if (wanted && (rc = dev_alloc_t(e, &op.xwin, t_floats(pl, tw.t[op.in].d_bf16)))) return rc;
                }
            } else {
                if ((rc = dev_alloc_t(e, &y.d, t_floats(y, y.d_bf16)))) return rc;
                if ((rc = dev_alloc_t(e, &y.g, t_floats(y, y.g_bf16)))) return rc;
            }
            const Tensor& x = tw.t[op.in];
            if (op.kind == OP_CONV) {
                if ((rc = dev_alloc_t(e, &op.wflip, (size_t)e->params[op.p_kernel].numel))) return rc;
                if (conv_wino_floats(op.geom) && (rc = dev_alloc_t(e, &op.wino_uf, conv_wino_floats(op.geom)))) return rc;
                {
                    const size_t sf = (size_t)conv_wino_stat_blocks_max(op.geom) * 2 * op.geom.Cout;
                    if (sf > stat_max) stat_max = sf;
                    const size_t sb = (size_t)conv_bf16_stat_blocks(op.geom) * 2 * op.geom.Cout;
                    if (e->cfg.dtype == L3_DTYPE_BF16 && sb > stat_max) stat_max = sb;
                    const size_t s1 = (size_t)conv_first_stat_blocks(op.geom) * 2 * op.geom.Cout;
                    if (s1 > stat_max) stat_max = s1;
                    const size_t sd = op.dy_to_bn >= 0 ? (size_t)conv_wino_stat_blocks_max(op.dgeom) * 2 * op.dgeom.Cout : 0;
                    if (sd > stat_max) stat_max = sd;
                    const size_t sdb = op.dy_to_bn >= 0 && e->cfg.dtype == L3_DTYPE_BF16
                                           ? (size_t)conv_bf16_stat_blocks(op.dgeom) * 2 * op.dgeom.Cout : 0;
                    if (sdb > stat_max) stat_max = sdb;
                }
                if (op.need_dx && conv_wino_floats(op.dgeom) &&
                    (rc = dev_alloc_t(e, &op.wino_ud, conv_wino_floats(op.dgeom))))
                    return rc;
                const size_t w = conv_wgrad_scratch_floats(op.geom);
                if (w > wg_max) wg_max = w;
                if (op.in_bn >= 0) {
                    if ((rc = dev_alloc_t(e, &op.xaug, (size_t)x.rows() * op.ageom.Cin))) return rc;
                    if ((rc = dev_alloc_t(e, &op.gaug, (size_t)op.kh * op.kw * op.ageom.Cin * op.cout))) return rc;
                    const size_t wa = conv_wgrad_scratch_floats(op.ageom);
                    if (wa > wg_max) wg_max = wa;
                }
                const size_t r = colreduce_scratch_floats(y.rows(), y.C);
                if (r > red_max) red_max = r;
            } else if (op.kind == OP_BN) {
                const int C = x.C;
                for (float** p : {&op.mean, &op.var, &op.scale, &op.shift, &op.biased_mean, &op.biased_var}) {
                    if ((rc = dev_alloc_t(e, p, (size_t)(C + 3) / 4 * 4))) return rc;
                    HIPCHK(e, hipMemset(*p, 0, (size_t)(C + 3) / 4 * 4 * 4));
                }
                const size_t r = colreduce_scratch_floats(x.rows(), C);
                if (r > red_max) red_max = r;
            }
        }
    }
    if (e->vis.ops.back().kind != OP_POOL || e->aud.ops.back().kind != OP_POOL) {
        e->err = "tower must end in a pooling layer";
        return L3_EINVAL;
    }
    if ((rc = dev_alloc_t(e, &e->red_scratch, red_max))) return rc;
    if ((rc = dev_alloc_t(e, &e->wg_scratch, wg_max))) return rc;
    if ((rc = dev_alloc_t(e, &e->sq_scratch, 2048))) return rc;
    if (stat_max && (rc = dev_alloc_t(e, &e->stat_scratch, stat_max))) return rc;
    {
        bool any_w4 = false;
        for (Tower* tw : {&e->vis, &e->aud})
            for (auto& op : tw->ops)
                if (op.kind == OP_CONV && (op.wino_uf || op.wino_ud)) any_w4 = true;
        if (any_w4 && e->cfg.dtype != L3_DTYPE_BF16 && (rc = dev_alloc_t(e, &e->w4_tail, conv_wino4_tail_scratch_bytes() / sizeof(float)))) return rc;
    }
    if (e->side) {
        if ((rc = dev_alloc_t(e, &e->red_scratch2, red_max))) return rc;
        if ((rc = dev_alloc_t(e, &e->wg_scratch2, wg_max))) return rc;
        if (stat_max && (rc = dev_alloc_t(e, &e->stat_scratch2, stat_max))) return rc;
    }
    return L3_OK;
}

int run_frontend(l3_engine* e) {
    int rc = rebuild_consts(e);
    if (rc) return rc;
    const FrontendCfg& f = e->fcfg;
    const int B = e->B;
    const int M = B * f.n_frames;
    const bool mag = e->cfg.frontend == L3_FRONTEND_MINISPEC && f.n_mels > 0;
    if (f.factored) {
        const int N1 = f.N1, N2 = f.N2;
        const int form = knob_int("L3_DFT_FACTORED", 1);
        if (form != 2 && f.n_mels > 0 && N1 == 32 && N2 == 64) {
            const double m1 = (double)M * N2, m2 = (double)M * N1;
            ProfScope ps(e, F_FRONTEND, 2.0 * M * (double)f.n_dft * 2.0 * f.n_freq + 2.0 * M * (double)f.n_freq * f.n_mels, nullptr,
                         2.0 * m1 * N1 * 2 * N1 + 2.0 * m2 * 2 * N2 * N2);
            dft_fused(e->audio, e->dft_win, e->dft_b1, e->dft_b2, e->dft_tw, e->melw, e->mel_start, e->mel_len, e->mel_off, e->aud.t[0].d, B,
                      AUDIO_T, f, e->stream, mag);
            if (f.db) db_normalize(e->aud.t[0].d, e->smax, B, e->aud.t[0].batch_stride, e->cfg.db_max_scope, e->stream);
            return L3_OK;
        }
        {
            ProfScope ps(e, F_FRONTEND, 0.0);
            dft_pack_frames(e->audio, e->dft_win, e->frames, B, AUDIO_T, f, e->stream);
        }
        {
            const double m1 = (double)M * N2, m2 = (double)M * N1;
            ProfScope ps(e, F_FRONTEND, 2.0 * M * (double)f.n_dft * 2.0 * f.n_freq, nullptr, 2.0 * m1 * N1 * 2 * N1 + 2.0 * m2 * 2 * N2 * N2);
            const ConvGeom g1{1, 1, M * N2, N1, 1, M * N2, 2 * N1, 1, 1, 0, 0}, g2{1, 1, M * N1, 2 * N2, 1, M * N1, N2, 1, 1, 0, 0};
            conv_fwd(e->frames, e->dft_b1, nullptr, e->dft_y, g1, e->stream);
            dft_twiddle(e->dft_y, e->dft_tw, e->dft_a2, e->dft_nyq, M, f, e->stream);
            conv_fwd(e->dft_a2, e->dft_b2, nullptr, e->spec, g2, e->stream);
        }
    } else if (f.folded) {
        float* fe = e->frames;
        float* fo = e->frames + (size_t)M * f.ke;
        {
            ProfScope ps(e, F_FRONTEND, 0.0);
            frame_audio_folded(e->audio, fe, fo, B, AUDIO_T, f, e->stream);
        }
        ProfScope ps(e, F_FRONTEND, 2.0 * M * (double)f.n_dft * 2.0 * f.n_freq, nullptr,
                     2.0 * M * (double)(f.ke + f.ko) * f.nc);
        const ConvGeom ge{1, 1, M, f.ke, 1, M, f.nc, 1, 1, 0, 0}, go{1, 1, M, f.ko, 1, M, f.nc, 1, 1, 0, 0};
        conv_fwd(fe, e->wdft, nullptr, e->spec, ge, e->stream);
        conv_fwd(fo, e->wdft + (size_t)f.ke * f.nc, nullptr, e->spec + (size_t)M * f.nc, go, e->stream);
    } else {
        {
            ProfScope ps(e, F_FRONTEND, 0.0);
            frame_audio(e->audio, e->frames, B, AUDIO_T, f, e->stream);
        }
        ConvGeom g{1, 1, M, f.n_dft, 1, M, f.ncols_pad, 1, 1, 0, 0};
        ProfScope ps(e, F_FRONTEND, 2.0 * M * (double)f.n_dft * 2.0 * f.n_freq);
        conv_fwd(e->frames, e->wdft, nullptr, e->spec, g, e->stream);
    }
    {
        ProfScope ps(e, F_FRONTEND, f.n_mels ? 2.0 * B * f.n_frames * (double)f.n_freq * f.n_mels : 0.0);
        spec_to_features(e->spec, e->melw, e->mel_start, e->mel_len, e->mel_off, e->aud.t[0].d, B, f, e->stream, e->dft_nyq, mag);
        if (f.db) db_normalize(e->aud.t[0].d, e->smax, B, e->aud.t[0].batch_stride, e->cfg.db_max_scope, e->stream);
    }
    return L3_OK;
}

static inline double act_bytes(const Tensor& t) { return (double)t.numel() * (t.d_bf16 ? 2.0 : 4.0); }
static inline double grad_bytes(const Tensor& t) { return (double)t.numel() * (t.g_bf16 ? 2.0 : 4.0); }

int plan_tower(l3_engine* e, Tower& tw, bool training, int solo) {
    static const int epi_stats = knob_int("L3_EPILOGUE_STATS", 1);
    const bool bf16 = e->cfg.dtype == L3_DTYPE_BF16;
    tw.training = training;
    auto fits = [&](const Op& cv, int blocks, int C) {
        if ((size_t)blocks * 2 * C <= e->stat_max) return true;
        e->err = cv.name + ": " + std::to_string(blocks) + " partial blocks of " + std::to_string(C) + " channels exceed the statistics scratch (" +
                 std::to_string(e->stat_max) + " floats)";
        return false;
    };
    auto defers = [&](const Op& bn) {
        return training && bn.defer_apply && bn.fuse_pool < 0 && bn_fast_ok(tw.t[bn.in].C) && tw.t[bn.in].d_bf16 == tw.t[bn.out].g_bf16;
    };
    for (auto& op : tw.ops) op.bp = BnPlan{};
    for (auto& op : tw.ops) {
        if (op.kind != OP_CONV) continue;
        op.geom.solo = op.dgeom.solo = solo;
        op.geom.dynamic = op.dgeom.dynamic = e->comm != nullptr ? 1 : 0;
        float* ts = solo ? e->w4_tail : nullptr;
        op.geom.tail_scratch = op.dgeom.tail_scratch = ts;
        op.geom.tail_scratch_bytes = op.dgeom.tail_scratch_bytes = ts ? conv_wino4_tail_scratch_bytes() : 0;

        const Tensor &x = tw.t[op.in], &y = tw.t[op.out];
        const double wbytes = (double)e->params[op.p_kernel].numel * 4.0;
        ConvPlan& p = op.cp = ConvPlan{};
        p.st = ConvStorage{bf16, x.d_bf16, y.d_bf16, y.g_bf16, x.g_bf16};
        p.fwd = conv_resolve_fwd(op.geom, p.st, op.wino_uf != nullptr);
        p.fwd_bytes = act_bytes(x) + act_bytes(y) + wbytes;
        const int nblk = conv_fwd_stat_blocks(p.fwd, op.geom);
        if (epi_stats && training && op.bn_follow >= 0 && e->stat_max > 0 && nblk > 0) {
            if (!fits(op, nblk, op.geom.Cout)) return L3_ESTATE;
            p.stat_mode = tw.ops[op.bn_follow].prerelu ? 2 : 1;
            tw.ops[op.bn_follow].bp.stat_blocks = nblk;
        }
        if (training && op.in_bn >= 0) {
            const Op* fb = op.bn_defer >= 0 && defers(tw.ops[op.bn_defer]) ? &tw.ops[op.bn_defer] : nullptr;
            p.aug = fb ? FW_AUG_DEFERRED : FW_AUG;
            p.wg_bytes = (double)x.rows() * op.ageom.Cin * 4.0 + (fb ? act_bytes(tw.t[fb->in]) + grad_bytes(tw.t[fb->out]) : grad_bytes(y));
            continue;
        }
        p.wgrad = conv_resolve_wgrad(op.geom, p.st);
        p.wg_bytes = act_bytes(x) + grad_bytes(y) + wbytes;
        p.colsum = !op.bias_by_bn;
        if (!op.need_dx) continue;
        p.dgrad = conv_resolve_dgrad(op.geom, op.dgeom, p.st, op.wino_ud != nullptr);
        p.dg_bytes = grad_bytes(y) + grad_bytes(x) + wbytes;
        Op* bn = training && op.dy_to_bn >= 0 && e->stat_max > 0 ? &tw.ops[op.dy_to_bn] : nullptr;
        if (bn != nullptr && bn->fuse_pool >= 0 && (bn->xwin == nullptr || x.batch_stride != (int64_t)x.H * x.W * x.C)) bn = nullptr;
        if (bn == nullptr) continue;
        const int blocks = conv_dgrad_bn_blocks(p.dgrad, op.dgeom, x.g_bf16, tw.t[bn->in].d_bf16);
        if (blocks < 0) continue;
        if (!fits(op, blocks, op.dgeom.Cout)) return L3_ESTATE;
        p.bwd_bn = op.dy_to_bn;
        bn->bp.bwd_blocks = blocks;
    }
    for (auto& op : tw.ops) {
        if (op.kind != OP_BN) continue;
        const Tensor &x = tw.t[op.in], &y = tw.t[op.out];
        const Tensor& out = op.fuse_pool >= 0 ? tw.t[tw.ops[op.fuse_pool].out] : y;
        BnPlan& p = op.bp;
        p.stats = !training ? BS_MOVING : p.stat_blocks > 0 ? BS_PARTIALS : op.prerelu || x.d_bf16 ? BS_FAST : BS_PLAIN;
        p.bwd = training && op.fused_first ? BB_BY_FIRST_CONV : !bn_fast_ok(x.C) ? BB_PLAIN : op.fuse_pool >= 0 ? BB_FAST_POOLED
                : defers(op) ? BB_FAST_DEFERRED : BB_FAST;
        p.fwd_bytes = (!training ? 0.0 : p.stat_blocks > 0 ? (double)p.stat_blocks * 2 * x.C * 4 : act_bytes(x)) + act_bytes(x) + act_bytes(out);
        if (p.bwd == BB_BY_FIRST_CONV) p.fwd_bytes += act_bytes(x) + (double)x.rows() * (&op + 1)->ageom.Cin * 4.0;
        if (op.fuse_pool >= 0 && training && op.xwin != nullptr) p.fwd_bytes += (double)out.numel() * (x.d_bf16 ? 2.0 : 4.0);
        p.bwd_bytes = p.bwd == BB_PLAIN ? 2.0 * (act_bytes(x) + grad_bytes(y)) + grad_bytes(x)
                                        : (p.bwd_blocks > 0 ? (double)p.bwd_blocks * 2 * x.C * 4 : act_bytes(x) + grad_bytes(out)) +
                                              (p.bwd == BB_FAST_DEFERRED ? 0.0 : act_bytes(x) + grad_bytes(out) + grad_bytes(x));
    }
    return L3_OK;
}

void tower_forward(l3_engine* e, Tower& tw) {
    const bool training = tw.training;
    for (auto& op : tw.ops) {
        Tensor& x = tw.t[op.in];
        Tensor& y = tw.t[op.out];
        switch (op.kind) {
            case OP_CONV: {
                const ConvPlan& p = op.cp;
                ConvBufs b;
                b.x = x.d, b.w = e->params[op.p_kernel].d, b.bias = e->params[op.p_bias].d, b.y = y.d;
                b.wprep = op.wflip, b.wino_u = op.wino_uf;
                b.stat_part = p.stat_mode ? e->stat_scratch : nullptr, b.stat_mode = p.stat_mode;
                ProfScope ps(e, F_CONV_FWD, conv_flops(op.geom), op.name.c_str(), p.fwd.executed);
                ps.bytes(p.fwd_bytes);
                conv_run_fwd(p.fwd, op.geom, p.st, b, e->stream);
                break;
            }
            case OP_BN: {
                const BnPlan& p = op.bp;
                ProfScope ps(e, F_ELEMWISE, 0.0);
                ps.bytes(p.fwd_bytes);
                const float* gamma = e->params[op.p_gamma].d;
                const float* beta = e->params[op.p_beta].d;
                switch (p.stats) {
                    case BS_PARTIALS:
                        bn_stats_from_partials(e->stat_scratch, p.stat_blocks, e->params[op.bias_param].d, gamma, beta, op.mean, op.var,
                                               op.scale, op.shift, x.rows(), x.C, BN_EPS, op.prerelu ? 1 : 0, e->stream);
                        break;
                    case BS_FAST:
                        bn_stats_fast(x.d, gamma, beta, op.mean, op.var, op.scale, op.shift, e->red_scratch, x.rows(), x.C, BN_EPS,
                                      op.prerelu ? 1 : 0, e->stream, x.d_bf16 ? 1 : 0);
                        break;
                    case BS_PLAIN:
                        bn_stats(x.d, gamma, beta, op.mean, op.var, op.scale, op.shift, e->red_scratch, x.rows(), x.C, BN_EPS, e->stream);
                        break;
                    case BS_MOVING:
                        bn_scale_shift(gamma, beta, e->params[op.p_mmean].d, e->params[op.p_mvar].d, op.scale, op.shift, x.C, BN_EPS,
                                       e->stream);
                        break;
                }
                if (p.bwd == BB_BY_FIRST_CONV) bn_xhat_ones(x.d, op.mean, op.var, BN_EPS, (&op + 1)->xaug, x.rows(), x.C, e->stream);
                if (op.fuse_pool >= 0) {
                    Tensor& pl = tw.t[tw.ops[op.fuse_pool].out];
                    bn_relu_pool2_fwd(x.d, op.scale, op.shift, pl.d, x.N, x.H, x.W, x.C, pl.H, pl.W, pl.batch_stride,
                                      op.prerelu ? 2 : (op.fused_relu ? 1 : 0), e->stream, pl.d_bf16 ? 1 : 0, x.d_bf16 ? 1 : 0,
                                      training ? (void*)op.xwin : nullptr);
                } else if (y.d_bf16 || x.d_bf16) {
                    bn_apply_fast(x.d, op.scale, op.shift, y.d, x.rows(), x.C, op.fused_relu ? 1 : 0, e->stream, y.d_bf16 ? 1 : 0,
                                  x.d_bf16 ? 1 : 0);
                } else {
                    bn_apply(x.d, op.scale, op.shift, y.d, x.rows(), x.C, op.fused_relu ? 1 : 0, e->stream);
                }
                break;
            }
            case OP_RELU: {
                if (op.fused_into_bn) break;
                ProfScope ps(e, F_ELEMWISE, 0.0);
                ps.bytes(act_bytes(x) + act_bytes(y));
                relu_fwd(x.d, y.d, x.numel(), e->stream);
                break;
            }
            case OP_POOL: {
                if (op.fused_into_bn) break;
                ProfScope ps(e, F_ELEMWISE, 0.0);
                ps.bytes(act_bytes(x) + act_bytes(y));
                maxpool_fwd(x.d, y.d, op.pg, e->stream);
                break;
            }
            default: break;
        }
    }
}

BnBwdFuse bn_bwd_fuse(const Tower& tw, const Op& bn) {
    return BnBwdFuse{bn.fuse_pool >= 0 ? bn.xwin : tw.t[bn.in].d, bn.scale, bn.shift, bn.mean, bn.var, BN_EPS, bn.fused_relu ? 1 : 0};
}

void tower_backward_block(l3_engine* e, Tower& tw, int block) {
    const bool training = tw.training;
    for (int oi = (int)tw.ops.size() - 1; oi >= 0; --oi) {
        Op& op = tw.ops[oi];
        if (op.block != block) continue;
        Tensor& x = tw.t[op.in];
        Tensor& y = tw.t[op.out];
        switch (op.kind) {
            case OP_POOL: {
                if (op.fused_into_bn) break;
                ProfScope ps(e, F_ELEMWISE, 0.0);
                ps.bytes(act_bytes(x) + grad_bytes(y) + grad_bytes(x));
                maxpool_bwd(x.d, y.g, x.g, op.pg, e->stream);
                break;
            }
            case OP_RELU: {
                if (op.fused_into_bn) break;
                ProfScope ps(e, F_ELEMWISE, 0.0);
                ps.bytes(act_bytes(y) + grad_bytes(y) + grad_bytes(x));
                relu_bwd(y.d, y.g, x.g, x.numel(), e->stream);
                break;
            }
            case OP_BN: {
                const BnPlan& p = op.bp;
                if (p.bwd == BB_BY_FIRST_CONV) break;
                ProfScope ps(e, F_ELEMWISE, 0.0);
                ps.bytes(p.bwd_bytes);
                const float* mean = training ? op.mean : e->params[op.p_mmean].d;
                const float* var = training ? op.var : e->params[op.p_mvar].d;
                const float* gamma = e->params[op.p_gamma].d;
                float *dgamma = e->params[op.p_gamma].g, *dbeta = e->params[op.p_beta].g;
                if (p.bwd == BB_PLAIN) {
                    bn_bwd(x.d, y.d, y.g, gamma, mean, var, x.g, dgamma, dbeta, e->red_scratch, x.rows(), x.C, BN_EPS, op.fused_relu ? 1 : 0,
                           training ? 1 : 0, e->stream);
                    break;
                }
                const bool pooled = p.bwd == BB_FAST_POOLED, defer = p.bwd == BB_FAST_DEFERRED;
                const Tensor& dy = pooled ? tw.t[tw.ops[op.fuse_pool].out] : y;
                bn_bwd_fast(x.d, op.scale, op.shift, mean, var, gamma, dy.g, pooled ? 1 : 0, x.N, x.H, x.W, x.C, dy.H, dy.W,
                            pooled ? dy.batch_stride : (int64_t)x.H * x.W * x.C, defer ? nullptr : x.g, dgamma, dbeta,
                            defer ? nullptr : op.bias_param >= 0 ? e->params[op.bias_param].g : nullptr, e->red_scratch, BN_EPS,
                            pooled ? (op.prerelu ? 2 : 1) : (op.fused_relu ? 1 : 0), training ? 1 : 0, e->stream, x.g_bf16 ? 1 : 0,
                            x.d_bf16 ? 1 : 0, dy.g_bf16 ? 1 : 0, p.bwd_blocks > 0 ? e->stat_scratch : nullptr, p.bwd_blocks);
                break;
            }
            case OP_CONV: {
                const ConvPlan& p = op.cp;
                const float* w = e->params[op.p_kernel].d;
                if (p.aug != FW_NONE) {
                    ProfScope ps(e, F_CONV_WGRAD, conv_flops(op.geom), op.name.c_str());
                    ps.bytes(p.wg_bytes);
                    const Op& bn = tw.ops[op.in_bn];
                    if (p.aug == FW_AUG_DEFERRED) {
                        const Op& fb = tw.ops[op.bn_defer];
                        const Tensor &bi = tw.t[fb.in], &bo = tw.t[fb.out];
                        const float* co = bn_bwd_fast_coeffs(e->red_scratch, op.cout);
                        const FirstWgFuse f{bi.d, bo.g, fb.scale, fb.shift, co, co + op.cout, co + 2 * op.cout, fb.fused_relu ? 1 : 0,
                                            bi.d_bf16 ? 1 : 0};
                        conv_wgrad(op.xaug, nullptr, op.gaug, e->wg_scratch, op.ageom, e->stream, false, false, &f);
                    } else {
                        conv_wgrad(op.xaug, y.g, op.gaug, e->wg_scratch, op.ageom, e->stream);
                    }
                    first_conv_grads(op.gaug, w, e->params[bn.p_gamma].d, e->params[bn.p_beta].d, e->params[op.p_kernel].g,
                                     e->params[bn.p_gamma].g, e->params[bn.p_beta].g,
                                     op.bias_by_bn && p.aug == FW_AUG ? nullptr : e->params[op.p_bias].g, op.kh * op.kw, x.C, op.cout,
                                     e->stream);
                    break;
                }
                ConvBufs b;
                b.x = x.d, b.w = w, b.y = y.g, b.dx = x.g, b.dw = e->params[op.p_kernel].g;
                b.wprep = op.wflip, b.wino_u = op.wino_ud, b.wg_part = e->wg_scratch;
                {
                    ProfScope ps(e, F_CONV_WGRAD, conv_flops(op.geom), op.name.c_str(), p.wgrad.executed);
                    ps.bytes(p.wg_bytes);
                    conv_run_wgrad(p.wgrad, op.geom, b, e->stream);
                }
                if (p.colsum) {
                    ProfScope ps(e, F_ELEMWISE, 0.0);
                    ps.bytes(grad_bytes(y));
                    colsum(y.g, e->params[op.p_bias].g, e->red_scratch, y.rows(), y.C, e->stream);
                }
                if (p.dgrad.path == DG_NONE) break;
                ProfScope ps(e, F_CONV_DGRAD, conv_flops(op.geom), op.name.c_str(), p.dgrad.executed);
                ps.bytes(p.dg_bytes);
                BnBwdFuse bb{};
                if (p.bwd_bn >= 0) {
                    bb = bn_bwd_fuse(tw, tw.ops[p.bwd_bn]);
                    b.bn_bwd = &bb, b.stat_part = e->stat_scratch;
                }
                conv_run_dgrad(p.dgrad, op.geom, op.dgeom, p.st, b, e->stream);
                break;
            }
            default: break;
        }
    }
}

void l2_sums(l3_engine* e) {
    SumsqSegs segs{};
    int nl2 = 0;
    for (auto& s : e->segments) nl2 += s.l2 ? 1 : 0;
    if (nl2 <= SUMSQ_MAX_SEGS) {
        for (auto& s : e->segments)
            if (s.l2) {
                segs.off[segs.count] = s.off;
                segs.n[segs.count++] = s.n;
            }
        sumsq_multi(e->arena_p, segs, e->l2part, e->sq_scratch, e->stream);
        return;
    }
    int si = 0;
    for (auto& s : e->segments)
        if (s.l2) sumsq(e->arena_p + s.off, s.n, e->l2part + si++, e->sq_scratch, e->stream);
}

int forward_all(l3_engine* e, bool training) {
    int rc;
// ... 1690 lines not shown
    if ((rc = embed_dest_check(e, fn, dst, n_frames, D))) return rc;
    int64_t bad = 0;
    if (const char* why = resample_clips_error(clips, n_clips, n_native, AUDIO_T, n_window, num_table, n_samples, true, &bad)) {
        e->err = name + ": " + (bad >= 0 ? "clip " + std::to_string(bad) + ": " : std::string()) + why;
        return L3_EINVAL;
    }
    if (const char* why = frame_table_error(table, n_frames, n_samples, &bad)) {
        e->err = name + ": frame " + std::to_string(bad) + ": " + why;
        return L3_EINVAL;
    }
    if (n_frames == 0) return L3_OK;
    HIPCHK(e, hipSetDevice(e->cfg.device));
    if ((rc = dev_grow_t(e, &e->clip_samples, &e->clip_samples_cap, (size_t)(n_samples > 0 ? n_samples : 1)))) return rc;
    if ((rc = dev_grow_t(e, &e->clip_table, &e->clip_table_cap, (size_t)n_frames * 3))) return rc;
    if ((rc = e->resample.run(native, n_native, clips, n_clips, AUDIO_T, half_window, n_window, num_table, true, e->clip_samples,
                              n_samples, e->stream, &e->err)))
        return rc;
    HIPCHK(e, hipMemcpyAsync(e->clip_table, table, (size_t)n_frames * 3 * 8, hipMemcpyHostToDevice, e->stream));
    EmbedSource src;
    src.samples = e->clip_samples;
    src.table = e->clip_table;
    return embed_rows(e, false, src, n_frames, pool_h, pool_w, D, dst);
}

int l3_embed_audio_clips_resampled(l3_engine* e, const float* native, int64_t n_native, const int64_t* clips, int64_t n_clips,
                                   const double* half_window, int64_t n_window, int num_table, int64_t n_samples,
                                   const int64_t* table, int64_t n_frames, int pool_h, int pool_w, float* out) {
    if (!e) return L3_EINVAL;
    EmbedDest dst;
    dst.host = out;
    return embed_clips_resampled_to(e, "l3_embed_audio_clips_resampled", native, n_native, clips, n_clips, half_window, n_window,
                                    num_table, n_samples, table, n_frames, pool_h, pool_w, dst);
}

int l3_embed_audio_clips_resampled_dev(l3_engine* e, const float* native, int64_t n_native, const int64_t* clips, int64_t n_clips,
                                       const double* half_window, int64_t n_window, int num_table, int64_t n_samples,
                                       const int64_t* table, int64_t n_frames, int pool_h, int pool_w, l3_feat* dst_feat,
                                       int64_t row0) {
    if (!e) return L3_EINVAL;
    EmbedDest dst;
    dst.dev = true, dst.feat = dst_feat, dst.row0 = row0;
    return embed_clips_resampled_to(e, "l3_embed_audio_clips_resampled_dev", native, n_native, clips, n_clips, half_window, n_window,
                                    num_table, n_samples, table, n_frames, pool_h, pool_w, dst);
}

int l3_activation_numel(l3_engine* e, const char* name, int64_t* numel) {
    if (!e || !name || !numel) return L3_EINVAL;
    const std::string nm(name);
    if (nm == "h0") { *numel = (int64_t)e->B * (e->nv + e->na); return L3_OK; }
    if (nm == "h1") { *numel = (int64_t)e->B * e->head; return L3_OK; }
    if (nm == "logits" || nm == "probs") { *numel = (int64_t)e->B * 2; return L3_OK; }
    Tensor* t = nullptr;
    if (!find_tower_tensor(e, nm, &t)) {
        e->err = "unknown activation: " + nm;
        return L3_EINVAL;
    }
    *numel = t->numel();
    return L3_OK;
}

int l3_get_activation(l3_engine* e, const char* name, float* dst, int64_t numel) {
    int64_t n = 0;
    int rc = l3_activation_numel(e, name, &n);
    if (rc) return rc;
    if (n != numel) {
        e->err = "activation size mismatch";
        return L3_EINVAL;
    }
    HIPCHK(e, hipSetDevice(e->cfg.device));
    HIPCHK(e, l3::stream_wait(e->stream));
    const std::string nm(name);
    const float* src = nullptr;
    if (nm == "h0") src = e->h0;
    else if (nm == "h1") src = e->h1;
    else if (nm == "logits") src = e->logits;
    else if (nm == "probs") src = e->probs;
    else {
        Tensor* t = nullptr;
        find_tower_tensor(e, nm, &t);
        if (t->alias || t->d == nullptr) {
            e->err = "activation is not materialised (aliased into h0 or fused away)";
            return L3_EINVAL;
        }
        src = t->d;
        if (t->d_bf16) {
            std::vector<uint16_t> h((size_t)numel);
            HIPCHK(e, hipMemcpy(h.data(), src, (size_t)numel * 2, hipMemcpyDeviceToHost));
            l3::widen_bf16(dst, h.data(), (size_t)numel);
            return L3_OK;
        }
    }
    HIPCHK(e, hipMemcpy(dst, src, (size_t)numel * 4, hipMemcpyDeviceToHost));
    return L3_OK;
}

int l3_sync(l3_engine* e) {
    if (!e) return L3_EINVAL;
    HIPCHK(e, hipSetDevice(e->cfg.device));
    HIPCHK(e, l3::stream_wait(e->stream));
    if (e->side) HIPCHK(e, l3::stream_wait(e->side));
    prof_collect(e);
    return L3_OK;
}

int l3_set_tower_overlap(l3_engine* e, int on) {
    if (!e) return L3_EINVAL;
    HIPCHK(e, l3::stream_wait(e->stream));
    if (e->side) HIPCHK(e, l3::stream_wait(e->side));
    e->overlap = on != 0;
    return L3_OK;
}

int l3_profile_enable(l3_engine* e, int on) {
    if (!e) return L3_EINVAL;
    HIPCHK(e, l3::stream_wait(e->stream));
    if (e->side) HIPCHK(e, l3::stream_wait(e->side));
    prof_collect(e);
    e->prof_on = on != 0;
    if (on)
        for (int i = 0; i < F_COUNT; ++i) {
            e->prof_ms[i] = 0;
            e->prof_n[i] = 0;
            e->prof_flops[i] = 0;
            e->prof_exec[i] = 0;
            e->prof_bytes[i] = 0;
        }
    return L3_OK;
}

int l3_profile_read(l3_engine* e, int family, double* ms, int64_t* launches, double* flops) {
    if (!e || family < 0 || family >= F_COUNT) return L3_EINVAL;
    HIPCHK(e, l3::stream_wait(e->stream));
    prof_collect(e);
    if (ms) *ms = e->prof_ms[family];
    if (launches) *launches = e->prof_n[family];
    if (flops) *flops = e->prof_flops[family];
    return L3_OK;
}

int l3_profile_read_bytes(l3_engine* e, int family, double* bytes) {
    if (!e || !bytes || family < 0 || family >= F_COUNT) return L3_EINVAL;
    HIPCHK(e, l3::stream_wait(e->stream));
    prof_collect(e);
    *bytes = e->prof_bytes[family];
    return L3_OK;
}

int l3_profile_read_executed(l3_engine* e, int family, double* flops) {
    if (!e || !flops || family < 0 || family >= F_COUNT) return L3_EINVAL;
    HIPCHK(e, l3::stream_wait(e->stream));
    prof_collect(e);
    *flops = e->prof_exec[family];
    return L3_OK;
}

}
```

### l3embedding_amd/csrc/kernels.h

```cpp
#pragma once
#include <hip/hip_runtime.h>
#include <stdint.h>

#include <string>
#include <vector>

#include "host_common.h"

struct l3_clipbank;
struct l3_sample;

namespace l3 {

struct ConvGeom {
    int N, H, W, Cin;
    int Ho, Wo, Cout;
    int KH, KW, padT, padL;
    int f2x2 = 0;
    int solo = 0;
    int dynamic = 0;
    float* tail_scratch = nullptr;
    size_t tail_scratch_bytes = 0;
};
size_t conv_wino4_tail_scratch_bytes();
// ... 29 lines not shown
bool conv_first_wgrad_ok(const ConvGeom& g);
size_t conv_first_wgrad_scratch_floats(const ConvGeom& g);
struct FirstWgFuse {
    const void *bnx, *dA;
    const float *scale, *shift;
    const float *cA, *cB, *cC;
    int relu;
    int bf16;
};
int conv_first_wgrad(const float* x, const float* dy, float* part, const ConvGeom& g, hipStream_t s, const FirstWgFuse* fuse = nullptr);
int conv_first_stat_blocks(const ConvGeom& g);
void conv_first_fwd(const float* x, const float* w, const float* bias, void* y, const ConvGeom& g, hipStream_t s,
                    float* stat_part = nullptr, int stat_mode = 0, bool out_bf16 = false);

bool conv_wgrad_wino_ok(const ConvGeom& g);
int conv_wgrad_wino_splits(const ConvGeom& g, int n);
int conv_wgrad_wino_max_splits(const ConvGeom& g, int n);
double conv_wgrad_wino_executed_flops(const ConvGeom& g);
void conv_wgrad_wino_launch(const float* x, const float* dy, float* part, const ConvGeom& g, int n, hipStream_t s);
void conv_wgrad_wino_finish(const float* part, float* dw, const ConvGeom& g, int splits, hipStream_t s);
double conv_wgrad_executed_flops(const ConvGeom& g, bool bf16);
bool conv_wgrad_bf16_tr_enabled();
void conv_wgrad_bf16_tr_launch(const void* x, const void* dy, float* part, const ConvGeom& g, int n, int splits, hipStream_t s);

bool conv_bf16_ok(const ConvGeom& g);
void conv_bf16_fwd(const float* x, const float* wn, const float* bias, float* y, const ConvGeom& g, hipStream_t s,
                   bool operands_bf16 = false, float* stat_part = nullptr, int stat_mode = 0, bool out_bf16 = false,
                   const BnBwdFuse* bn_bwd = nullptr);
int conv_bf16_stat_blocks(const ConvGeom& g);
bool conv_bf16_halo_ok(const ConvGeom& g);
int conv_bf16_halo_patches(const ConvGeom& g, int n);
void conv_bf16_halo_launch(const void* x, const void* wn, const float* bias, void* y, const ConvGeom& g, int n,
                           hipStream_t s, float* stat_part, int stat_mode, bool out_bf16, const BnBwdFuse* bn_bwd = nullptr);
void conv_weights_bf16(const float* w, void* out, int KH, int KW, int Cin, int Cout, bool flip, hipStream_t s);

void bn_xhat_ones(const float* x, const float* mean, const float* var, float eps, float* xa, int64_t rows, int C,
                  hipStream_t s);
void first_conv_grads(const float* gaug, const float* w, const float* gamma, const float* beta, float* dw, float* dgamma,
                      float* dbeta, float* dbias, int taps, int C, int Co, hipStream_t s);

size_t colreduce_scratch_floats(int64_t rows, int C);
void colsum(const float* x, float* out, float* scratch, int64_t rows, int C, hipStream_t s);
void bn_stats(const float* x, const float* gamma, const float* beta, float* mean, float* var,
              float* scale, float* shift, float* scratch, int64_t rows, int C, float eps,
              hipStream_t s);
void bn_scale_shift(const float* gamma, const float* beta, const float* mean, const float* var,
                    float* scale, float* shift, int C, float eps, hipStream_t s);
void bn_apply(const float* x, const float* scale, const float* shift, float* y, int64_t rows, int C,
              int relu, hipStream_t s);
void bn_bwd(const float* x, const float* y, const float* dy, const float* gamma, const float* mean,
            const float* var, float* dx, float* dgamma, float* dbeta, float* scratch, int64_t rows,
            int C, float eps, int relu, int training, hipStream_t s);
void bn_moving_update(float* moving, float* biased, const float* batch, int C, float momentum,
                      int zero_debias, int step, hipStream_t s);
int* persistent_work_counters(hipStream_t s);

struct BnMovingEntry {
    float* moving;
    float* biased;
    const float* batch;
    int C;
    int off;
};
void bn_moving_update_all(const BnMovingEntry* tab_dev, int entries, int max_c, float momentum, int zero_debias, int64_t step,
                          hipStream_t s, const float* gathered = nullptr, int replicas = 1, int64_t stride = 0);
void bn_moving_pack(const BnMovingEntry* tab_dev, int entries, int max_c, float* packed, hipStream_t s);

bool bn_fast_ok(int C);
size_t bn_fast_scratch_floats(int C);
void bn_stats_fast(const float* x, const float* gamma, const float* beta, float* mean, float* var, float* scale,
                   float* shift, float* scratch, int64_t rows, int C, float eps, int prerelu, hipStream_t s, int x_bf16 = 0);
void bn_stats_from_partials(const float* part, int nblk, const float* pivot, const float* gamma, const float* beta,
                            float* mean, float* var, float* scale, float* shift, int64_t rows, int C, float eps,
                            int prerelu, hipStream_t s);
void bn_apply_fast(const float* x, const float* scale, const float* shift, float* y, int64_t rows, int C, int relu,
                   hipStream_t s, int out_bf16 = 0, int x_bf16 = 0);
void bn_relu_pool2_fwd(const float* x, const float* scale, const float* shift, float* p, int N, int H, int W, int C,
                       int Ho, int Wo, int64_t out_batch_stride, int mode, hipStream_t s, int out_bf16 = 0, int x_bf16 = 0,
                       void* xwin = nullptr);
void bn_bwd_fast(const float* x, const float* scale, const float* shift, const float* mean, const float* var,
                 const float* gamma, const float* dy, int pooled, int N, int H, int W, int C, int Ho, int Wo,
                 int64_t dy_batch_stride, float* dx, float* dgamma, float* dbeta, float* dbias, float* scratch,
                 float eps, int relu, int training, hipStream_t s, int dx_bf16 = 0, int x_bf16 = 0, int dy_bf16 = 0,
                 const float* ready_part = nullptr, int ready_blocks = 0);
const float* bn_bwd_fast_coeffs(const float* scratch, int C);

void relu_fwd(const float* x, float* y, int64_t n, hipStream_t s);
void relu_bwd(const float* y, const float* dy, float* dx, int64_t n, hipStream_t s);

struct PoolGeom {
    int N, H, W, C, Ho, Wo, ph, pw, sh, sw, padT, padL;
    int64_t out_batch_stride;
};
void maxpool_fwd(const float* x, float* y, const PoolGeom& g, hipStream_t s);
void maxpool_bwd(const float* x, const float* dy, float* dx, const PoolGeom& g, hipStream_t s);

void preprocess_video(const uint8_t* u8, float* out, int64_t n, hipStream_t s);
void preprocess_audio(const int16_t* pcm, float* out, int64_t n, hipStream_t s);
void labels_onehot(const int32_t* lab, float* out, int64_t n, hipStream_t s);

struct AugmentParams {
    int32_t start_x, start_y, flip, sat_first;
    float saturation, brightness;
};
constexpr int AUG_CROP = 224;
void augment_video(const uint8_t* u8, int N, int H, int W, const AugmentParams* params, uint8_t* out_u8, float* out_f32,
                   hipStream_t s);
void augment_audio(const int16_t* pcm, int N, int T, const double* u, int16_t* out_i16, float* out_f32, double* gains,
                   hipStream_t s);

struct FrontendCfg {
    int n_dft, n_hop, pad_left, n_frames, n_freq, n_mels;
    int sqrt_out;
    int db;
    int loglambda;
    int ncols_pad;
    int folded, ke, ko, nc;
    int factored, N1, N2;
};
void dft_pack_frames(const float* audio, const float* win, float* a1, int B, int T, const FrontendCfg& c, hipStream_t s);
void dft_twiddle(const float* y, const float* tw, float* a2, float* nyq, int frames, const FrontendCfg& c, hipStream_t s);
void frame_audio_folded(const float* audio, float* fe, float* fo, int B, int T, const FrontendCfg& c, hipStream_t s);
void frame_audio(const float* audio, float* frames, int B, int T, const FrontendCfg& c, hipStream_t s);
void dft_fused(const float* audio, const float* win, const float* b1, const float* b2, const float* tw, const float* melw,
               const int* mel_start, const int* mel_len, const int* mel_off, float* out, int B, int T, const FrontendCfg& c,
               hipStream_t s, bool mag = false);
void spec_to_features(const float* spec, const float* melw, const int* mel_start, const int* mel_len,
                      const int* mel_off, float* out, int B, const FrontendCfg& c, hipStream_t s, const float* nyq = nullptr,
                      bool mag = false);
void db_normalize(float* x, float* smax, int B, int64_t per_sample, int batch_scope, hipStream_t s);
FrontendCfg frontend_cfg(int T, int n_dft, int n_hop, bool same, int n_mels, int sqrt_out, int db, int loglambda);
void host_mel_basis(int sr, int n_fft, int n_mels, std::vector<float>& freq2mel);
struct DftTables {
    std::vector<float> win, b1, b2, tw;
};
void dft_factor_tables(int n_dft, int N1, int N2, DftTables& t);
struct MelBands {
    std::vector<int> start, len, off;
    std::vector<float> w;
};
void mel_pack_bands(const float* fb, int nb, int n_mels, MelBands& m);

void gather_frames(const float* samples, const int64_t* table, float* out, int rows, int n_real, int T, hipStream_t s);
inline const char* frame_table_error(const int64_t* table, int64_t n_frames, int64_t n_samples, int64_t* bad_row) {
    const int64_t lim = (int64_t)1 << 62;
    for (int64_t r = 0; r < n_frames; ++r) {
        const int64_t start = table[3 * r], lo = table[3 * r + 1], hi = table[3 * r + 2];
        *bad_row = r;
        if (lo < 0) return "lo < 0";
        if (lo > hi) return "lo > hi";
        if (hi > n_samples) return "hi > n_samples";
        if (start < -lim || start > lim) return "start out of range";
    }
    return nullptr;
}

constexpr int IMG = 224;
constexpr int IMAGE_ROW = 7;
constexpr int IMAGE_DESC = 4;
constexpr int64_t IMAGE_MAX_SIDE = 8192;
const char* image_table_error(const int64_t* table, int64_t n_frames, int64_t n_bytes, int64_t* bad_row);
struct ImagePlan {
    std::vector<int64_t> frames, taps;
};
void image_plan(const int64_t* table, int64_t n_frames, ImagePlan* plan);
void image_frames(const uint8_t* pixels, const int64_t* frames, const int64_t* taps, uint8_t* out_u8, float* out_f32, int rows,
                  int n_real, hipStream_t s);

constexpr int SAMPLE_T = 48000;
constexpr int DOWNMIX_MAX_CHANNELS = 8;
void audio_downmix(const int16_t* in, int16_t* out, int64_t n, int C, hipStream_t s);
void audio_seconds(const int16_t* samples, const int64_t* table, int16_t* out, int rows, int T, hipStream_t s);
struct SampledHost {
    std::vector<int64_t> table, seconds;
    ImagePlan plan;
    std::vector<int32_t> labels;
    std::vector<AugmentParams> params;
// ... 118 lines not shown
```

### l3embedding_amd/csrc/ops.hip

```cpp
#include <hip/hip_runtime.h>

#include <cstring>
#include <string>
#include <vector>

#include "../../include/l3hip.h"
#include "conv_path.h"
#include "kernels.h"
#include "knobs.h"
#include "mlp.h"
#include "vggish.h"

namespace {
using namespace l3;

struct Scope {
    DeviceBufs bufs;
    hipStream_t s = nullptr;
    bool ok = true;
    explicit Scope(int device) : ok(device_ok(device)) {}
    ~Scope() { (void)hipDeviceSynchronize(); }
    template <class T>
    T* alloc(size_t count) {
        T* p = bufs.alloc<T>(count);
// ... 1593 lines not shown
            set_op_error("l3_op_vggish_conv1: example " + std::to_string(e) + " outside the log-mel rows");
            return L3_EINVAL;
        }
    if (n_examples == 0) return L3_OK;
    Scope sc(device);
    if (int rc = vggish_op_device("l3_op_vggish_conv1", sc, device)) return rc;
    const float* d_l = sc.put(logmel, (size_t)n_rows * VG_MELS);
    const int64_t* d_e = sc.put(example_rows, (size_t)n_examples);
    const float* d_w = sc.put(w, 9 * 64);
    const float* d_b = sc.put(b, 64);
    const size_t ny = (size_t)n_examples * (VG_ROWS / 2) * (VG_MELS / 2) * 64;
    float* d_y = sc.alloc<float>(ny);
    if (!sc.ok) return L3_ENOMEM;
    vggish_conv1(d_l, d_e, d_w, d_b, d_y, (int)n_examples, sc.s);
    sc.get(y, d_y, ny);
    return sc.status();
}

extern "C" int l3_op_vggish_bias_relu(int device, const float* x, const float* b, float* y, int n, int h, int wd, int c, int pool) {
    if (!x || !b || !y || n <= 0 || h <= 0 || wd <= 0 || c <= 0 || c % 4 != 0 || (pool && (h % 2 != 0 || wd % 2 != 0))) {
        set_op_error("l3_op_vggish_bias_relu: NULL pointer, c not a multiple of 4, or an odd map under the pool");
        return L3_EINVAL;
    }
    Scope sc(device);
    if (int rc = vggish_op_device("l3_op_vggish_bias_relu", sc, device)) return rc;
    const size_t nx = (size_t)n * h * wd * c, ny = pool ? nx / 4 : nx;
    const float* d_x = sc.put(x, nx);
    const float* d_b = sc.put(b, (size_t)c);
    float* d_y = sc.alloc<float>(ny);
    if (!sc.ok) return L3_ENOMEM;
    vggish_bias_relu(d_x, d_b, d_y, n, h, wd, c, pool ? 1 : 0, sc.s);
    sc.get(y, d_y, ny);
    return sc.status();
}

extern "C" int l3_op_vggish_postprocess(int device, const float* emb, int64_t n, const float* pca_matrix, const float* pca_means,
                                        int quantize, float* out) {
    if (!emb || !pca_matrix || !pca_means || !out || n <= 0 || n > (1 << 24)) {
        set_op_error("l3_op_vggish_postprocess: NULL pointer or bad count");
        return L3_EINVAL;
    }
    Scope sc(device);
    if (int rc = vggish_op_device("l3_op_vggish_postprocess", sc, device)) return rc;
    std::vector<float> t((size_t)VG_EMB * VG_EMB);
    for (int j = 0; j < VG_EMB; ++j)
        for (int k = 0; k < VG_EMB; ++k) t[(size_t)k * VG_EMB + j] = pca_matrix[(size_t)j * VG_EMB + k];
    const float* d_e = sc.put(emb, (size_t)n * VG_EMB);
    const float* d_p = sc.put(t.data(), t.size());
    const float* d_m = sc.put(pca_means, (size_t)VG_EMB);
    float* d_o = sc.alloc<float>((size_t)n * VG_EMB);
    if (!sc.ok) return L3_ENOMEM;
    vggish_postprocess(d_e, d_p, d_m, d_o, (int)n, quantize ? 1 : 0, sc.s);
    sc.get(out, d_o, (size_t)n * VG_EMB);
    return sc.status();
}

extern "C" int l3_op_vggish_conv(int device, int fp32_conv, const float* x, const float* w, const float* b, float* y, int n, int h,
                                 int wd, int cin, int cout, int pool) {
    if (!x || !w || !b || !y || n <= 0 || h <= 0 || wd <= 0 || cin <= 0 || cout <= 0 || cout % 4 != 0 ||
        (pool && (h % 2 != 0 || wd % 2 != 0)) ||
        (fp32_conv != L3_FP32_CONV_F4X4 && fp32_conv != L3_FP32_CONV_F2X2 && fp32_conv != L3_VGGISH_CONV_DIRECT)) {
        set_op_error("l3_op_vggish_conv: NULL pointer, bad size, cout not a multiple of 4, an odd map under the pool, or a bad fp32_conv");
        return L3_EINVAL;
    }
    Scope sc(device);
    if (int rc = vggish_op_device("l3_op_vggish_conv", sc, device)) return rc;
    ConvGeom g = conv_geom(n, h, wd, cin, cout, 3, 3, true, fp32_conv == L3_FP32_CONV_F2X2 ? 1 : 0);
    g.solo = 1;
    const ConvFwdPath p = conv_resolve_fwd(g, ConvStorage{}, fp32_conv != L3_VGGISH_CONV_DIRECT);
    const size_t nx = (size_t)n * h * wd * cin, nc = (size_t)n * h * wd * cout, ny = pool ? nc / 4 : nc;
    ConvBufs cb;
    cb.x = sc.put(x, nx);
    cb.w = sc.put(w, (size_t)9 * cin * cout);
    const float* d_b = sc.put(b, (size_t)cout);
    cb.wino_u = p.wino_filter ? sc.alloc<float>(conv_wino_floats(g)) : nullptr;
    float* d_c = cb.y = sc.alloc<float>(nc);
    float* d_y = sc.alloc<float>(ny);
    if (!sc.ok) return L3_ENOMEM;
    conv_run_fwd(p, g, ConvStorage{}, cb, sc.s);
    vggish_bias_relu(d_c, d_b, d_y, n, h, wd, cout, pool ? 1 : 0, sc.s);
    sc.get(y, d_y, ny);
    return sc.status();
}
```

Baseline: 2036 pairs/s.

## Fuse final BN+ReLU with global max pool and sparse winner-based backward

```diff
diff --git a/include/l3hip.h b/include/l3hip.h
--- a/include/l3hip.h
+++ b/include/l3hip.h
@@ -188,6 +188,12 @@
 int l3_op_bn_relu_pool2_bwd(int device, const float *x, const float *gamma, const float *beta, const float *dp,
                             float *dx, float *dgamma, float *dbeta, float *dbias, int n, int h, int wd, int c,
                             int same, int relu_mode, int x_bf16);
+int l3_op_bn_relu_gpool_fwd(int device, const float *x, const float *gamma, const float *beta, float *p, int32_t *win,
+                            float *mean, float *var, int n, int h, int wd, int c, int relu_mode, int64_t out_stride,
+                            int64_t out_off);
+int l3_op_bn_relu_gpool_bwd(int device, const float *x, const float *gamma, const float *beta, const float *mean,
+                            const float *var, const int32_t *win, const float *g, float *dx, float *dgamma, float *dbeta,
+                            float *dbias, int n, int h, int wd, int c, int relu_mode, int64_t g_stride, int64_t g_off);
 int l3_op_maxpool_fwd(int device, const float *x, float *y, int n, int h, int wd, int c,
                       int ph, int pw, int sh, int sw, int same);
 int l3_op_maxpool_bwd(int device, const float *x, const float *dy, float *dx, int n, int h,
diff --git a/l3embedding_amd/_lib.py b/l3embedding_amd/_lib.py
--- a/l3embedding_amd/_lib.py
+++ b/l3embedding_amd/_lib.py
@@ -150,6 +150,8 @@
     'l3_op_bn_relu_bwd': (C.c_int, [C.c_int] + [C.c_void_p] * 10 + [C.c_int64, C.c_int, C.c_int, C.c_int]),
     'l3_op_bn_relu_pool2_fwd': (C.c_int, [C.c_int] + [C.c_void_p] * 6 + [C.c_int] * 7),
     'l3_op_bn_relu_pool2_bwd': (C.c_int, [C.c_int] + [C.c_void_p] * 8 + [C.c_int] * 7),
+    'l3_op_bn_relu_gpool_fwd': (C.c_int, [C.c_int] + [C.c_void_p] * 7 + [C.c_int] * 5 + [C.c_int64] * 2),
+    'l3_op_bn_relu_gpool_bwd': (C.c_int, [C.c_int] + [C.c_void_p] * 11 + [C.c_int] * 5 + [C.c_int64] * 2),
     'l3_op_maxpool_fwd': (C.c_int, [C.c_int, C.c_void_p, C.c_void_p] + [C.c_int] * 9),
     'l3_op_maxpool_bwd': (C.c_int, [C.c_int, C.c_void_p, C.c_void_p, C.c_void_p] + [C.c_int] * 9),
     'l3_op_frontend': (C.c_int, [C.c_int, C.c_int, C.c_void_p, C.c_int, C.c_int, C.c_void_p]),
@@ -1005,6 +1007,33 @@
     return dx, dg, db, dbias
 
 
+def op_bn_relu_gpool_fwd(x, gamma, beta, p, col, device=0, relu_mode=1, want_win=True):
+    lib = load()
+    x = _f32(x)
+    n, h, wd, c = x.shape
+    if p.dtype != np.float32 or not p.flags['C_CONTIGUOUS'] or p.ndim != 2 or p.shape[0] != n:
+        raise ValueError('p must be a C-contiguous float32 array of n rows')
+    win = np.empty((n, c), np.int32) if want_win else None
+    mean, var = np.empty((c,), np.float32), np.empty((c,), np.float32)
+    check(lib.l3_op_bn_relu_gpool_fwd(device, _ptr(x), _ptr(_f32(gamma)), _ptr(_f32(beta)), _ptr(p), None if win is None else _ptr(win),
+                                      _ptr(mean), _ptr(var), n, h, wd, c, int(relu_mode), p.shape[1], int(col)))
+    return win, mean, var
+
+
+def op_bn_relu_gpool_bwd(x, gamma, beta, mean, var, win, g, col, device=0, relu_mode=1):
+    lib = load()
+    x, g = _f32(x), _f32(g)
+    n, h, wd, c = x.shape
+    win = np.ascontiguousarray(win, np.int32)
+    if g.ndim != 2 or g.shape[0] != n or win.shape != (n, c):
+        raise ValueError('g must have n rows and win the shape (n, c)')
+    dx = np.empty_like(x)
+    dg, db, dbias = (np.empty((c,), np.float32) for _ in range(3))
+    check(lib.l3_op_bn_relu_gpool_bwd(device, _ptr(x), _ptr(_f32(gamma)), _ptr(_f32(beta)), _ptr(_f32(mean)), _ptr(_f32(var)), _ptr(win),
+                                      _ptr(g), _ptr(dx), _ptr(dg), _ptr(db), _ptr(dbias), n, h, wd, c, int(relu_mode), g.shape[1], int(col)))
+    return dx, dg, db, dbias
+
+
 def _pool_out(h, p, s, same):
     return -(-h // s) if same else (h - p) // s + 1
 
diff --git a/l3embedding_amd/csrc/bn_fused.hip b/l3embedding_amd/csrc/bn_fused.hip
--- a/l3embedding_amd/csrc/bn_fused.hip
+++ b/l3embedding_amd/csrc/bn_fused.hip
@@ -342,15 +342,111 @@
                        reinterpret_cast<const f32x4*>(shift), (void*)p, g, mode, out_bf16, xwin);
 }
 
+template <bool WIN>
+__global__ __launch_bounds__(FB) void bn_relu_gpool_fwd_kernel(const float* __restrict__ x, const f32x4* scale, const f32x4* shift,
+                                                              float* __restrict__ p, int* __restrict__ win, int P, int C,
+                                                              int64_t out_batch_stride, int mode) {
+    constexpr int U = 8;
+    __shared__ float sb[16][64];
+    __shared__ int sa[16][64];
+    const int cb = blockIdx.x % (C / 64), n = blockIdx.x / (C / 64);
+    const int cq = threadIdx.x & 15, pg = threadIdx.x >> 4;
+    const int C4 = C / 4, c4 = cb * 16 + cq;
+    const f32x4 sc = scale[c4], sh = shift[c4];
+    const f32x4* xb = reinterpret_cast<const f32x4*>(x) + (int64_t)n * P * C4 + c4;
+    float best[4];
+    int arg[4];
+#pragma unroll
+    for (int e = 0; e < 4; ++e) {
+        best[e] = -INFINITY;
+        arg[e] = 0x7fffffff;
+    }
+    for (int p0 = pg; p0 < P; p0 += 16 * U) {
+        f32x4 v[U];
+#pragma unroll
+        for (int u = 0; u < U; ++u)
+            if (p0 + 16 * u < P) v[u] = __builtin_nontemporal_load(xb + (int64_t)(p0 + 16 * u) * C4);
+#pragma unroll
+        for (int u = 0; u < U; ++u) {
+            const int px = p0 + 16 * u;
+            if (px >= P) continue;
+            f32x4 a = bn_pre(mode == 2 ? relu4(v[u]) : v[u], sc, sh);
+            if (mode == 1) a = relu4(a);
+#pragma unroll
+            for (int e = 0; e < 4; ++e)
+                if (a[e] > best[e] || arg[e] == 0x7fffffff) {
+                    best[e] = a[e];
+                    arg[e] = px;
+                }
+        }
+    }
+#pragma unroll
+    for (int e = 0; e < 4; ++e) {
+        sb[pg][cq * 4 + e] = best[e];
+        sa[pg][cq * 4 + e] = arg[e];
+    }
+    __syncthreads();
+    if (threadIdx.x < 64) {
+        const int t = threadIdx.x;
+        float b = sb[0][t];
+        int a = sa[0][t];
+        for (int k = 1; k < 16; ++k) {
+            const float vb = sb[k][t];
+            const int va = sa[k][t];
+            if (vb > b || (vb == b && va < a)) {
+                b = vb;
+                a = va;
+            }
+        }
+        p[(int64_t)n * out_batch_stride + cb * 64 + t] = b;
+        if constexpr (WIN) win[(int64_t)n * C + cb * 64 + t] = a;
+    }
+}
+
+bool bn_relu_gpool_ok(int C, int64_t out_batch_stride) { return bn_fast_ok(C) && C % 64 == 0 && out_batch_stride % 4 == 0; }
+
+void bn_relu_gpool_fwd(const float* x, const float* scale, const float* shift, float* p, int* win, int N, int P, int C,
+                       int64_t out_batch_stride, int mode, hipStream_t s) {
+    auto k = win != nullptr ? bn_relu_gpool_fwd_kernel<true> : bn_relu_gpool_fwd_kernel<false>;
+    hipLaunchKernelGGL(k, dim3(N * (C / 64)), dim3(FB), 0, s, x, reinterpret_cast<const f32x4*>(scale),
+                       reinterpret_cast<const f32x4*>(shift), p, win, P, C, out_batch_stride, mode);
+}
+
 struct BwdCoef {
     float *A, *B, *Cc;
 };
 
-template <bool POOL, bool XBF, bool DYBF>
+struct HotSrc {
+    const int* win;
+    int P;
+    int64_t g_stride;
+};
+struct HotWalk {
+    int n, pix, dn, dp;
+    __device__ __forceinline__ HotWalk(int64_t q0, int64_t stride, int C4, int P) {
+        const int64_t row = q0 / C4, step = stride / C4;
+        n = (int)(row / P); pix = (int)(row % P);
+        dn = (int)(step / P); dp = (int)(step % P);
+    }
+    __device__ __forceinline__ void next(int P) {
+        n += dn; pix += dp;
+        if (pix >= P) { pix -= P; ++n; }
+    }
+};
+__device__ __forceinline__ i32x4 hot_winners(const HotSrc& h, int n, int N, int C4, int c4) {
+    return reinterpret_cast<const i32x4*>(h.win)[(int64_t)(n < N ? n : N - 1) * C4 + c4];
+}
+__device__ __forceinline__ bool hot_any(i32x4 w, int pix) { return w.x == pix || w.y == pix || w.z == pix || w.w == pix; }
+__device__ __forceinline__ f32x4 hot_grad(const HotSrc& h, const void* g, i32x4 w, int n, int pix, int c4) {
+    const f32x4 gv = *reinterpret_cast<const f32x4*>(reinterpret_cast<const float*>(g) + (int64_t)n * h.g_stride + c4 * 4);
+    return f32x4{w.x == pix ? gv.x : 0.f, w.y == pix ? gv.y : 0.f, w.z == pix ? gv.z : 0.f, w.w == pix ? gv.w : 0.f};
+}
+
+template <bool POOL, bool XBF, bool DYBF, bool HOT = false>
 __global__ __launch_bounds__(FB) void bn_bwd_reduce_fast_kernel(const void* x, const void* dy, const f32x4* scale,
                                                                const f32x4* shift, const f32x4* mean,
                                                                const f32x4* var, float* part, int64_t n4,
-                                                               Pool2Geom g, float eps, int relu) {
+                                                               Pool2Geom g, float eps, int relu, HotSrc hot) {
     const int64_t q0 = (int64_t)blockIdx.x * FB + threadIdx.x;
     const int c4 = (int)(q0 % g.C4);
     const f32x4 sc = scale[c4], sh = shift[c4], mu = mean[c4];
@@ -358,7 +454,35 @@
     const f32x4 rs = {rsqrtf(vv.x + eps), rsqrtf(vv.y + eps), rsqrtf(vv.z + eps), rsqrtf(vv.w + eps)};
     f32x4 a0 = {0.f, 0.f, 0.f, 0.f}, a1 = {0.f, 0.f, 0.f, 0.f};
     const int64_t stride = (int64_t)gridDim.x * FB;
-    if constexpr (!POOL) {
+    if constexpr (HOT) {
+        constexpr int U = 8;
+        HotWalk walk(q0, stride, g.C4, hot.P);
+        for (int64_t q = q0; q < n4; q += stride * U) {
+            i32x4 ws[U];
+            int ns[U], ps[U];
+#pragma unroll
+            for (int u = 0; u < U; ++u) {
+                ns[u] = walk.n; ps[u] = walk.pix;
+                ws[u] = hot_winners(hot, walk.n, g.N, g.C4, c4);
+                walk.next(hot.P);
+            }
+#pragma unroll
+            for (int u = 0; u < U; ++u) {
+                if (q + u * stride >= n4 || !hot_any(ws[u], ps[u])) continue;
+                f32x4 xv = load_quad<XBF>(x, q + u * stride);
+                f32x4 d = hot_grad(hot, dy, ws[u], ns[u], ps[u], c4);
+                if (relu == 1) {
+                    const f32x4 pre = bn_pre(xv, sc, sh);
+                    d.x = pre.x > 0.f ? d.x : 0.f; d.y = pre.y > 0.f ? d.y : 0.f;
+                    d.z = pre.z > 0.f ? d.z : 0.f; d.w = pre.w > 0.f ? d.w : 0.f;
+                } else if (relu == 2) {
+                    xv = relu4(xv);
+                }
+                a0 += d;
+                a1 += d * ((xv - mu) * rs);
+            }
+        }
+    } else if constexpr (!POOL) {
         for (int64_t q = q0; q < n4; q += stride) {
             f32x4 xv = load_quad<XBF>(x, q);
             f32x4 d = load_quad<DYBF>(dy, q);
@@ -430,17 +554,39 @@
     }
 };
 
-template <bool POOL, bool XBF, bool DYBF>
+template <bool POOL, bool XBF, bool DYBF, bool HOT = false>
 __global__ __launch_bounds__(FB) void bn_bwd_apply_fast_kernel(const void* x, const void* dy, const f32x4* scale,
                                                               const f32x4* shift, const f32x4* cA, const f32x4* cB,
                                                               const f32x4* cC, void* dx, float* part, int64_t n4,
-                                                              Pool2Geom g, int relu, int obf) {
+                                                              Pool2Geom g, int relu, int obf, HotSrc hot) {
     const int64_t q0 = (int64_t)blockIdx.x * FB + threadIdx.x;
     const int c4 = (int)(q0 % g.C4);
     const f32x4 sc = scale[c4], sh = shift[c4], A = cA[c4], B = cB[c4], Cc = cC[c4];
     f32x4 a0 = {0.f, 0.f, 0.f, 0.f};
     const int64_t stride = (int64_t)gridDim.x * FB;
-    if constexpr (!POOL) {
+    if constexpr (HOT) {
+        HotWalk walk(q0, stride, g.C4, hot.P);
+        for (int64_t q = q0; q < n4; q += stride) {
+            const f32x4 xr = load_quad<XBF>(x, q);
+            f32x4 xv = xr;
+            f32x4 d = hot_grad(hot, dy, hot_winners(hot, walk.n, g.N, g.C4, c4), walk.n, walk.pix, c4);
+            walk.next(hot.P);
+            if (relu == 1) {
+                const f32x4 pre = bn_pre(xv, sc, sh);
+                d.x = pre.x > 0.f ? d.x : 0.f; d.y = pre.y > 0.f ? d.y : 0.f;
+                d.z = pre.z > 0.f ? d.z : 0.f; d.w = pre.w > 0.f ? d.w : 0.f;
+            } else if (relu == 2) {
+                xv = relu4(xv);
+            }
+            f32x4 o = A * d + (B * xv + Cc);
+            if (relu == 2) {
+                o.x = xr.x > 0.f ? o.x : 0.f; o.y = xr.y > 0.f ? o.y : 0.f;
+                o.z = xr.z > 0.f ? o.z : 0.f; o.w = xr.w > 0.f ? o.w : 0.f;
+            }
+            store_quad(dx, q, o, obf);
+            a0 += o;
+        }
+    } else if constexpr (!POOL) {
         for (int64_t q = q0; q < n4; q += stride) {
             const f32x4 xr = load_quad<XBF>(x, q);
             f32x4 xv = xr;
@@ -553,7 +699,8 @@
                  const float* gamma, const float* dy, int pooled, int N, int H, int W, int C, int Ho, int Wo,
                  int64_t dy_batch_stride, float* dx, float* dgamma, float* dbeta, float* dbias, float* scratch,
                  float eps, int relu, int training, hipStream_t s, int dx_bf16, int x_bf16, int dy_bf16,
-                 const float* ready_part, int ready_blocks) {
+                 const float* ready_part, int ready_blocks, const int* hot_win, int64_t hot_g_stride) {
+    const HotSrc hot{hot_win, H * W, hot_g_stride};
     const int64_t rows = (int64_t)N * H * W;
     const int64_t n4 = rows * (C / 4);
     Pool2Geom g = make_pool2(N, H, W, C, pooled ? Ho : H, pooled ? Wo : W, pooled ? dy_batch_stride : (int64_t)H * W * C);
@@ -569,7 +716,7 @@
     const int nb_r = fast_blocks(work_r);
     const int variant = (pooled ? 4 : 0) | (x_bf16 ? 2 : 0) | (dy_bf16 ? 1 : 0);
     using ReduceFn = void (*)(const void*, const void*, const f32x4*, const f32x4*, const f32x4*, const f32x4*, float*, int64_t,
-                              Pool2Geom, float, int);
+                              Pool2Geom, float, int, HotSrc);
     static const ReduceFn reduce_fns[8] = {
         bn_bwd_reduce_fast_kernel<false, false, false>, bn_bwd_reduce_fast_kernel<false, false, true>,
         bn_bwd_reduce_fast_kernel<false, true, false>,  bn_bwd_reduce_fast_kernel<false, true, true>,
@@ -579,8 +726,9 @@
         launch_fast_final(BwdFinal{gamma, mean, var, dgamma, dbeta, cA, cB, cC, 1.0 / (double)rows, eps, training}, ready_part,
                           ready_blocks, C, s);
     } else {
-        hipLaunchKernelGGL(reduce_fns[variant], dim3(nb_r), dim3(FB), 0, s, xv, dyv, sc4, sh4, reinterpret_cast<const f32x4*>(mean),
-                           reinterpret_cast<const f32x4*>(var), part, n4, g, eps, relu);
+        const ReduceFn rf = hot_win != nullptr ? bn_bwd_reduce_fast_kernel<false, false, false, true> : reduce_fns[variant];
+        hipLaunchKernelGGL(rf, dim3(nb_r), dim3(FB), 0, s, xv, dyv, sc4, sh4, reinterpret_cast<const f32x4*>(mean),
+                           reinterpret_cast<const f32x4*>(var), part, n4, g, eps, relu, hot);
         launch_fast_final(BwdFinal{gamma, mean, var, dgamma, dbeta, cA, cB, cC, 1.0 / (double)rows, eps, training}, part,
                           nb_r, C, s);
     }
@@ -589,15 +737,16 @@
     const int nb_a = fast_blocks(work_a);
     float* part2 = dbias ? part : nullptr;
     using ApplyFn = void (*)(const void*, const void*, const f32x4*, const f32x4*, const f32x4*, const f32x4*, const f32x4*, void*,
-                             float*, int64_t, Pool2Geom, int, int);
+                             float*, int64_t, Pool2Geom, int, int, HotSrc);
     static const ApplyFn apply_fns[8] = {
         bn_bwd_apply_fast_kernel<false, false, false>, bn_bwd_apply_fast_kernel<false, false, true>,
         bn_bwd_apply_fast_kernel<false, true, false>,  bn_bwd_apply_fast_kernel<false, true, true>,
         bn_bwd_apply_fast_kernel<true, false, false>,  bn_bwd_apply_fast_kernel<true, false, true>,
         bn_bwd_apply_fast_kernel<true, true, false>,   bn_bwd_apply_fast_kernel<true, true, true>};
-    hipLaunchKernelGGL(apply_fns[variant], dim3(nb_a), dim3(FB), 0, s, xv, dyv, sc4, sh4, reinterpret_cast<const f32x4*>(cA),
+    const ApplyFn af = hot_win != nullptr ? bn_bwd_apply_fast_kernel<false, false, false, true> : apply_fns[variant];
+    hipLaunchKernelGGL(af, dim3(nb_a), dim3(FB), 0, s, xv, dyv, sc4, sh4, reinterpret_cast<const f32x4*>(cA),
                        reinterpret_cast<const f32x4*>(cB), reinterpret_cast<const f32x4*>(cC), (void*)dx, part2, n4, g, relu,
-                       dx_bf16);
+                       dx_bf16, hot);
     if (dbias) launch_fast_final(SumFinal{dbias}, part, nb_a, C, s);
 }
 
diff --git a/l3embedding_amd/csrc/elementwise.hip b/l3embedding_amd/csrc/elementwise.hip
--- a/l3embedding_amd/csrc/elementwise.hip
+++ b/l3embedding_amd/csrc/elementwise.hip
@@ -552,6 +552,7 @@
     return g.Ho == 1 && g.Wo == 1 && g.padT == 0 && g.padL == 0 && g.ph == g.H && g.pw == g.W && g.C % 64 == 0 &&
            g.out_batch_stride % 4 == 0;
 }
+bool maxpool_is_global(const PoolGeom& g) { return is_global_pool(g); }
 
 void maxpool_fwd(const float* x, float* y, const PoolGeom& g, hipStream_t s) {
     if (is_global_pool(g)) {
diff --git a/l3embedding_amd/csrc/engine.hip b/l3embedding_amd/csrc/engine.hip
--- a/l3embedding_amd/csrc/engine.hip
+++ b/l3embedding_amd/csrc/engine.hip
@@ -73,6 +73,7 @@
     int stat_blocks = 0;
     BnBwd bwd = BB_PLAIN;
     int bwd_blocks = 0;
+    bool tower_end = false;
     double fwd_bytes = 0.0, bwd_bytes = 0.0;
 };
 
@@ -104,6 +105,8 @@
     int fuse_pool = -1;
     int bias_param = -1;
     bool fused_into_bn = false;
+    int* win = nullptr;
+    bool out_stale = false;
     bool bias_by_bn = false;
     float *mean = nullptr, *var = nullptr, *scale = nullptr, *shift = nullptr;
     float *biased_mean = nullptr, *biased_var = nullptr;
@@ -974,6 +977,16 @@
         e->err = "tower must end in a pooling layer";
         return L3_EINVAL;
     }
+    for (Tower* tw : {&e->vis, &e->aud}) {
+        const size_t L = tw->ops.size() - 1;
+        if (L < 1) continue;
+        Op &pool = tw->ops[L], &bn = tw->ops[L - 1];
+        const Tensor &x = tw->t[bn.in], &y = tw->t[bn.out];
+        if (bn.kind == OP_BN && bn.fused_relu && !bn.prerelu && bn.fuse_pool < 0 && !bn.fused_first && !bn.defer_apply &&
+            pool.in == bn.out && !pool.fused_into_bn && maxpool_is_global(pool.pg) && bn_relu_gpool_ok(x.C, pool.pg.out_batch_stride) &&
+            !x.d_bf16 && !y.d_bf16 && !x.g_bf16 && !y.g_bf16 && (rc = dev_alloc_t(e, &bn.win, (size_t)x.N * x.C)))
+            return rc;
+    }
     if ((rc = dev_alloc_t(e, &e->red_scratch, red_max))) return rc;
     if ((rc = dev_alloc_t(e, &e->wg_scratch, wg_max))) return rc;
     if ((rc = dev_alloc_t(e, &e->sq_scratch, 2048))) return rc;
@@ -1111,6 +1124,7 @@
         p.bwd_bn = op.dy_to_bn;
         bn->bp.bwd_blocks = blocks;
     }
+    const bool tower_end = knob_int("L3_TOWER_END", 1) != 0;
     for (auto& op : tw.ops) {
         if (op.kind != OP_BN) continue;
         const Tensor &x = tw.t[op.in], &y = tw.t[op.out];
@@ -1125,6 +1139,12 @@
         p.bwd_bytes = p.bwd == BB_PLAIN ? 2.0 * (act_bytes(x) + grad_bytes(y)) + grad_bytes(x)
                                         : (p.bwd_blocks > 0 ? (double)p.bwd_blocks * 2 * x.C * 4 : act_bytes(x) + grad_bytes(out)) +
                                               (p.bwd == BB_FAST_DEFERRED ? 0.0 : act_bytes(x) + grad_bytes(out) + grad_bytes(x));
+        if (tower_end && op.win != nullptr && p.bwd == BB_FAST && p.bwd_blocks == 0) {
+            p.tower_end = (&op + 1)->bp.tower_end = true;
+            const double row = (double)x.N * x.C * 4.0;
+            p.fwd_bytes += 2.0 * row - act_bytes(out);
+            p.bwd_bytes = 2.0 * (act_bytes(x) + 2.0 * row) + grad_bytes(x);
+        }
     }
     return L3_OK;
 }
@@ -1170,7 +1190,12 @@
                         break;
                 }
                 if (p.bwd == BB_BY_FIRST_CONV) bn_xhat_ones(x.d, op.mean, op.var, BN_EPS, (&op + 1)->xaug, x.rows(), x.C, e->stream);
-                if (op.fuse_pool >= 0) {
+                op.out_stale = p.tower_end;
+                if (p.tower_end) {
+                    const Op& pool = *(&op + 1);
+                    bn_relu_gpool_fwd(x.d, op.scale, op.shift, tw.t[pool.out].d, op.win, x.N, x.H * x.W, x.C, pool.pg.out_batch_stride, 1,
+                                      e->stream);
+                } else if (op.fuse_pool >= 0) {
                     Tensor& pl = tw.t[tw.ops[op.fuse_pool].out];
                     bn_relu_pool2_fwd(x.d, op.scale, op.shift, pl.d, x.N, x.H, x.W, x.C, pl.H, pl.W, pl.batch_stride,
                                       op.prerelu ? 2 : (op.fused_relu ? 1 : 0), e->stream, pl.d_bf16 ? 1 : 0, x.d_bf16 ? 1 : 0,
@@ -1191,7 +1216,7 @@
                 break;
             }
             case OP_POOL: {
-                if (op.fused_into_bn) break;
+                if (op.fused_into_bn || op.bp.tower_end) break;
                 ProfScope ps(e, F_ELEMWISE, 0.0);
                 ps.bytes(act_bytes(x) + act_bytes(y));
                 maxpool_fwd(x.d, y.d, op.pg, e->stream);
@@ -1215,7 +1240,7 @@
         Tensor& y = tw.t[op.out];
         switch (op.kind) {
             case OP_POOL: {
-                if (op.fused_into_bn) break;
+                if (op.fused_into_bn || op.bp.tower_end) break;
                 ProfScope ps(e, F_ELEMWISE, 0.0);
                 ps.bytes(act_bytes(x) + grad_bytes(y) + grad_bytes(x));
                 maxpool_bwd(x.d, y.g, x.g, op.pg, e->stream);
@@ -1240,6 +1265,14 @@
                 if (p.bwd == BB_PLAIN) {
                     bn_bwd(x.d, y.d, y.g, gamma, mean, var, x.g, dgamma, dbeta, e->red_scratch, x.rows(), x.C, BN_EPS, op.fused_relu ? 1 : 0,
                            training ? 1 : 0, e->stream);
+                    break;
+                }
+                if (p.tower_end) {
+                    const Op& pool = *(&op + 1);
+                    bn_bwd_fast(x.d, op.scale, op.shift, mean, var, gamma, tw.t[pool.out].g, 0, x.N, x.H, x.W, x.C, x.H, x.W,
+                                (int64_t)x.H * x.W * x.C, x.g, dgamma, dbeta, op.bias_param >= 0 ? e->params[op.bias_param].g : nullptr,
+                                e->red_scratch, BN_EPS, 1, training ? 1 : 0, e->stream, 0, 0, 0, nullptr, 0, op.win,
+                                pool.pg.out_batch_stride);
                     break;
                 }
                 const bool pooled = p.bwd == BB_FAST_POOLED, defer = p.bwd == BB_FAST_DEFERRED;
@@ -3096,6 +3129,14 @@
             e->err = "activation is not materialised (aliased into h0 or fused away)";
             return L3_EINVAL;
         }
+        for (Tower* tw : {&e->vis, &e->aud})
+            for (auto& op : tw->ops)
+                if (op.kind == OP_BN && op.out_stale && &tw->t[op.out] == t) {
+                    const Tensor& x = tw->t[op.in];
+                    bn_apply(x.d, op.scale, op.shift, t->d, x.rows(), x.C, op.fused_relu ? 1 : 0, e->stream);
+                    HIPCHK(e, l3::stream_wait(e->stream));
+                    op.out_stale = false;
+                }
         src = t->d;
         if (t->d_bf16) {
             std::vector<uint16_t> h((size_t)numel);
diff --git a/l3embedding_amd/csrc/kernels.h b/l3embedding_amd/csrc/kernels.h
--- a/l3embedding_amd/csrc/kernels.h
+++ b/l3embedding_amd/csrc/kernels.h
@@ -135,7 +135,12 @@
                  const float* gamma, const float* dy, int pooled, int N, int H, int W, int C, int Ho, int Wo,
                  int64_t dy_batch_stride, float* dx, float* dgamma, float* dbeta, float* dbias, float* scratch,
                  float eps, int relu, int training, hipStream_t s, int dx_bf16 = 0, int x_bf16 = 0, int dy_bf16 = 0,
-                 const float* ready_part = nullptr, int ready_blocks = 0);
+                 const float* ready_part = nullptr, int ready_blocks = 0,
+                 const int* hot_win = nullptr, int64_t hot_g_stride = 0);
+
+bool bn_relu_gpool_ok(int C, int64_t out_batch_stride);
+void bn_relu_gpool_fwd(const float* x, const float* scale, const float* shift, float* p, int* win, int N, int P, int C,
+                       int64_t out_batch_stride, int mode, hipStream_t s);
 const float* bn_bwd_fast_coeffs(const float* scratch, int C);
 
 void relu_fwd(const float* x, float* y, int64_t n, hipStream_t s);
@@ -146,6 +151,7 @@
     int64_t out_batch_stride;
 };
 void maxpool_fwd(const float* x, float* y, const PoolGeom& g, hipStream_t s);
+bool maxpool_is_global(const PoolGeom& g);
 void maxpool_bwd(const float* x, const float* dy, float* dx, const PoolGeom& g, hipStream_t s);
 
 void preprocess_video(const uint8_t* u8, float* out, int64_t n, hipStream_t s);
diff --git a/l3embedding_amd/csrc/ops.hip b/l3embedding_amd/csrc/ops.hip
--- a/l3embedding_amd/csrc/ops.hip
+++ b/l3embedding_amd/csrc/ops.hip
@@ -1699,3 +1699,102 @@
     sc.get(y, d_y, ny);
     return sc.status();
 }
+
+namespace {
+bool gpool_args_ok(const char* name, int n, int h, int wd, int c, int mode, int64_t stride, int64_t off) {
+    if (n >= 1 && h >= 1 && wd >= 1 && c >= 1 && mode >= 0 && mode <= 2 && stride >= 1 && bn_relu_gpool_ok(c, stride) && off >= 0 &&
+        off % 4 == 0 && off + c <= stride && (int64_t)n * h * wd < (int64_t)1 << 30 && (int64_t)n * stride < (int64_t)1 << 30)
+        return true;
+    set_op_error(std::string(name) + ": an empty shape, relu_mode outside 0..2, c not a power of two that is a multiple of 64, or a "
+                 "row stride / column offset that is not a multiple of 4 or does not hold c columns");
+    return false;
+}
+}
+
+extern "C" int l3_op_bn_relu_gpool_fwd(int device, const float* x, const float* gamma, const float* beta, float* p, int32_t* win,
+                                       float* mean, float* var, int n, int h, int wd, int c, int relu_mode, int64_t out_stride,
+                                       int64_t out_off) {
+    const char* name = "l3_op_bn_relu_gpool_fwd";
+    if (!x || !gamma || !beta || !p) return fail(L3_EINVAL, std::string(name) + ": NULL pointer");
+    if (!gpool_args_ok(name, n, h, wd, c, relu_mode, out_stride, out_off)) return L3_EINVAL;
+    Scope sc(device);
+    if (!sc.ok) return L3_EHIP;
+    const int P = h * wd;
+    const int64_t rows = (int64_t)n * P;
+    const size_t nx = (size_t)rows * c, np_ = (size_t)n * out_stride, nw = (size_t)n * c;
+    uint32_t nan_bits = 0x7fc00000u;
+    float nan;
+    memcpy(&nan, &nan_bits, sizeof nan);
+    std::vector<float> hp(p, p + np_);
+    for (int i = 0; i < n; ++i)
+        for (int k = 0; k < c; ++k) hp[(size_t)i * out_stride + out_off + k] = nan;
+    FeBufs fb(sc);
+    float* d_x = sc.put(x, nx);
+    float* d_g = sc.put(gamma, (size_t)c);
+    float* d_b = sc.put(beta, (size_t)c);
+    float *d_m = fb.fresh((size_t)c, "mean"), *d_v = fb.fresh((size_t)c, "var"), *d_sc = fb.fresh((size_t)c, "scale"),
+          *d_sh = fb.fresh((size_t)c, "shift");
+    float* d_p = fb.fresh(np_, "the pooled rows", hp.data());
+    int* d_win = win ? reinterpret_cast<int*>(fb.fresh(nw, "the winners")) : nullptr;
+    size_t red = colreduce_scratch_floats(rows, c);
+    if (bn_fast_scratch_floats(c) > red) red = bn_fast_scratch_floats(c);
+    float* d_red = fb.fresh(red, "the reduction scratch");
+    if (!sc.ok) return L3_ENOMEM;
+    if (relu_mode == 2)
+        bn_stats_fast(d_x, d_g, d_b, d_m, d_v, d_sc, d_sh, d_red, rows, c, 1e-3f, 1, sc.s, 0);
+    else
+        bn_stats(d_x, d_g, d_b, d_m, d_v, d_sc, d_sh, d_red, rows, c, 1e-3f, sc.s);
+    bn_relu_gpool_fwd(d_x, d_sc, d_sh, d_p + out_off, d_win, n, P, c, out_stride, relu_mode, sc.s);
+    if (const int rc = fb.check(name)) return rc;
+    sc.get(hp.data(), d_p, np_);
+    std::vector<int32_t> hw(win ? nw : 0);
+    if (win) sc.get(hw.data(), d_win, nw);
+    sc.get(mean, d_m, (size_t)c);
+    sc.get(var, d_v, (size_t)c);
+    if (!sc.ok) return L3_EHIP;
+    for (int i = 0; i < n; ++i)
+        for (int k = 0; k < c; ++k) {
+            const float v = hp[(size_t)i * out_stride + out_off + k];
+            if (v != v && relu_mode == 1)
+                return fail(L3_EINVAL, std::string(name) + ": column " + std::to_string(k) + " of row " + std::to_string(i) + " was not written");
+        }
+    for (size_t i = 0; i < hw.size(); ++i)
+        if (hw[i] < 0 || hw[i] >= P) return fail(L3_EINVAL, std::string(name) + ": winner " + std::to_string(i) + " was not written");
+    memcpy(p, hp.data(), np_ * sizeof(float));
+    if (win) memcpy(win, hw.data(), nw * sizeof(int32_t));
+    return sc.status();
+}
+
+extern "C" int l3_op_bn_relu_gpool_bwd(int device, const float* x, const float* gamma, const float* beta, const float* mean,
+                                       const float* var, const int32_t* win, const float* g, float* dx, float* dgamma, float* dbeta,
+                                       float* dbias, int n, int h, int wd, int c, int relu_mode, int64_t g_stride, int64_t g_off) {
+    const char* name = "l3_op_bn_relu_gpool_bwd";
+    if (!x || !gamma || !beta || !mean || !var || !win || !g || !dx || !dgamma || !dbeta) return fail(L3_EINVAL, std::string(name) + ": NULL pointer");
+    if (!gpool_args_ok(name, n, h, wd, c, relu_mode, g_stride, g_off)) return L3_EINVAL;
+    const int P = h * wd;
+    const size_t nx = (size_t)n * P * c, nw = (size_t)n * c;
+    for (size_t i = 0; i < nw; ++i)
+        if (win[i] < 0 || win[i] >= P) return fail(L3_EINVAL, std::string(name) + ": winner " + std::to_string(i) + " is no pixel of the image");
+    Scope sc(device);
+    if (!sc.ok) return L3_EHIP;
+    FeBufs fb(sc);
+    float* d_x = sc.put(x, nx);
+    float *d_g = sc.put(gamma, (size_t)c), *d_b = sc.put(beta, (size_t)c), *d_m = sc.put(mean, (size_t)c), *d_v = sc.put(var, (size_t)c);
+    int* d_win = sc.put(win, nw);
+    float* d_gr = sc.put(g, (size_t)n * g_stride);
+    float *d_sc = fb.fresh((size_t)c, "scale"), *d_sh = fb.fresh((size_t)c, "shift");
+    float* d_dx = fb.fresh(nx, "dx");
+    float *d_dg = fb.fresh((size_t)c, "dgamma"), *d_db = fb.fresh((size_t)c, "dbeta");
+    float* d_dbias = dbias ? fb.fresh((size_t)c, "dbias") : nullptr;
+    float* d_red = fb.fresh(bn_fast_scratch_floats(c), "the reduction scratch");
+    if (!sc.ok) return L3_ENOMEM;
+    bn_scale_shift(d_g, d_b, d_m, d_v, d_sc, d_sh, c, 1e-3f, sc.s);
+    bn_bwd_fast(d_x, d_sc, d_sh, d_m, d_v, d_g, d_gr + g_off, 0, n, h, wd, c, h, wd, (int64_t)P * c, d_dx, d_dg, d_db, d_dbias, d_red,
+                1e-3f, relu_mode, 1, sc.s, 0, 0, 0, nullptr, 0, d_win, g_stride);
+    if (const int rc = fb.check(name)) return rc;
+    sc.get(dx, d_dx, nx);
+    sc.get(dgamma, d_dg, (size_t)c);
+    sc.get(dbeta, d_db, (size_t)c);
+    sc.get(dbias, d_dbias, (size_t)c);
+    return sc.status();
+}
```

Result: no change. 2046 pairs/s (median of 6 runs) (+0.5%).
